# ZSHCRWY25/3DRVO-MARL-CollisionAvoidance

Measured on AMD Instinct MI355X. Metric: drone-steps/sec (env.step throughput), higher is better.
Workload: dtype f64; 1 GPU; BASELINE config 3 env.step: 64 drones x 4096 envs per GPU, nm=10, 0 buildings, map [50.0, 50.0, 10.0], fused step+auto-reset, f32 actions in HBM; envs_per_gpu=4096, drones=64, diag_build=False, cold_all=False, ablate=0, device_error_word=0

## Files before the change

### 3drvo-marl-collisionavoidance_amd/csrc/rvo3d_capi.hip

```cpp
#include "../../include/rvo3d.h"
#include "rvo3d_device.hpp"

#include <atomic>
#include <cmath>
#include <cstdio>
#include <cstdlib>
#include <cstring>
#include <exception>
#include <new>
#include <string>
#include <vector>

using rvo3d::Params;

namespace {
thread_local std::string g_err;

int fail(int code, const std::string& msg) {
  g_err = msg;
  return code;
}
#define HIP_TRY(expr)                                                            \
  do {                                                                           \
    hipError_t _e = (expr);                                                      \
    if (_e != hipSuccess)                                                        \
      return fail(RVO3D_ERR_HIP, std::string(#expr) + ": " + hipGetErrorString(_e)); \
  } while (0)

int api_caught(const char* what) noexcept {
  try {
    g_err = std::string("C++ exception: ") + what;
  } catch (...) {
    try { g_err.clear(); } catch (...) { }
  }
  return RVO3D_ERR_INVALID;
}
#define RVO3D_API_BEGIN try {
#define RVO3D_API_END                                              \
  }                                                                \
  catch (const std::exception& e) { return api_caught(e.what()); } \
  catch (...) { return api_caught("unknown"); }

inline size_t align_up(size_t x, size_t a) { return (x + a - 1) / a * a; }
volatile double kTwo = 2.0;
inline double py_sq(double x) { return std::pow(x, kTwo); }

double sq_threshold(double tau) {
  volatile double x = tau * tau;
  while (std::sqrt(std::nextafter((double)x, INFINITY)) <= tau) x = std::nextafter((double)x, INFINITY);
  while (std::sqrt((double)x) > tau) x = std::nextafter((double)x, -INFINITY);
  return x;
}
}

struct rvo3d_env {
  rvo3d_config cfg;
  Params P;
  rvo3d::Cold cold;
  void* arena = nullptr;
  size_t arena_bytes = 0;
  bool world_loaded = false;
  bool dv_valid = false;
  bool g_valid = false;
  int threads = 0, blocks = 0, lds = 0;
};

namespace {

int carve(rvo3d_env* h) {
  const rvo3d_config& c = h->cfg;
  const size_t EN = (size_t)c.num_envs * c.num_drones;
  const size_t S = align_up(EN, 64);
  Params& P = h->P;
  rvo3d::Cold& C = h->cold;
  P.S = (uint32_t)S;
  const size_t nf = Params::f64_arrays(c.max_points, c.neighbors_num);
  const size_t ni = Params::i32_arrays(c.neighbors_num, P.nw);
  struct Field { void** slot; size_t bytes; };
  std::vector<Field> f = {
      {(void**)&P.f64, nf * S * 8},
      {(void**)&P.i32, ni * S * 4},
      {(void**)&P.u8, 2 * S},
      {(void**)&C.bld, (size_t)(c.num_buildings > 0 ? c.num_buildings : 1) * 4 * 8},
      {(void**)&C.pow95, (size_t)c.max_points * 8},
      {(void**)&C.bgrid, (size_t)(C.bgx > 0 ? C.bgx * C.bgy : 1) * (rvo3d::kBgridK + 1) * 2},
      {(void**)&P.err, 256},
      {(void**)&P.cold_, sizeof(rvo3d::Cold)},
  };
  size_t total = 0;
  for (auto& x : f) total += align_up(x.bytes, 256);
  HIP_TRY(hipMalloc(&h->arena, total));
  HIP_TRY(hipMemset(h->arena, 0, total));
  h->arena_bytes = total;
  size_t off = 0;
  for (auto& x : f) {
    *x.slot = static_cast<char*>(h->arena) + off;
    off += align_up(x.bytes, 256);
  }
  HIP_TRY(hipMemcpy((void*)P.cold_, &C, sizeof C, hipMemcpyHostToDevice));
  return RVO3D_OK;
}

struct DeviceGuard {
  int prev = -1;
  bool changed = false;
  int enter(int dev) {
    hipError_t e = hipGetDevice(&prev);
    if (e == hipSuccess && prev != dev) {
      e = hipSetDevice(dev);
      changed = e == hipSuccess;
    }
    if (e != hipSuccess) return fail(RVO3D_ERR_HIP, std::string("hipSetDevice: ") + hipGetErrorString(e));
    return RVO3D_OK;
  }
  ~DeviceGuard() {
    if (changed) (void)hipSetDevice(prev);
  }
};

int check(rvo3d_env* h, bool need_world, DeviceGuard& g) {
  if (!h) return fail(RVO3D_ERR_INVALID, "null handle");
  if (need_world && !h->world_loaded)
    return fail(RVO3D_ERR_STATE, "rvo3d_load_world has not been called");
  return g.enter(h->cfg.device);
}

struct Pick { int nfix; bool pad; };
Pick pick_kernel(const Params& P) {
  if (P.nw == 1) {
    const int seg = (P.epb == 1 || P.epb == 2 || P.epb == 4) ? 64 / P.epb : 0;
    if (seg && P.N == seg) return {seg, false};
    if (seg >= 32 && P.N < seg) return {seg, true};
    return {0, false};
  }
  if (P.nw == 2) return {128, true};
  if (P.nw == 3) return {192, true};
  if (P.nw == 4) return {256, true};
  return {0, false};
}

template <int MODE, int NW, int NFIX, bool TRAIN, bool PAD>
void launch_inst(rvo3d_env* h, const Params& P, hipStream_t s) {
  hipLaunchKernelGGL((rvo3d::env_kernel<MODE, NW, NFIX, TRAIN, PAD>), dim3(h->blocks), dim3(h->threads), h->lds, s, P);
}
template <int MODE, int NW, int NFIX, bool PAD>
void launch_train(rvo3d_env* h, const Params& P, hipStream_t s) {
  if (P.env_train) launch_inst<MODE, NW, NFIX, true, PAD>(h, P, s);
  else launch_inst<MODE, NW, NFIX, false, PAD>(h, P, s);
}

template <int MODE, int NW>
int launch_nw(rvo3d_env* h, const Params& P, hipStream_t s) {
  const Pick k = pick_kernel(P);
  if constexpr (NW == 1) {
    if (k.nfix == 64) { if (k.pad) launch_train<MODE, 1, 64, true>(h, P, s); else launch_train<MODE, 1, 64, false>(h, P, s); }
    else if (k.nfix == 32) { if (k.pad) launch_train<MODE, 1, 32, true>(h, P, s); else launch_train<MODE, 1, 32, false>(h, P, s); }
    else if (k.nfix == 16) launch_train<MODE, 1, 16, false>(h, P, s);
    else launch_train<MODE, 1, 0, false>(h, P, s);
  } else if constexpr (NW == 2 || NW == 3 || NW == 4) {
    launch_train<MODE, NW, 64 * NW, true>(h, P, s);
  } else {
    launch_train<MODE, NW, 0, false>(h, P, s);
  }
  HIP_TRY(hipGetLastError());
  return RVO3D_OK;
}

template <int MODE>
int launch(rvo3d_env* h, const Params& P, hipStream_t s) {
  switch (P.nw) {
    case 1: return launch_nw<MODE, 1>(h, P, s);
    case 2: return launch_nw<MODE, 2>(h, P, s);
    case 3: return launch_nw<MODE, 3>(h, P, s);
    case 4: return launch_nw<MODE, 4>(h, P, s);
    default: return launch_nw<MODE, 8>(h, P, s);
  }
}

template <int MODE, int NW>
hipError_t allow_lds(int bytes) {
  hipError_t e = hipFuncSetAttribute((const void*)rvo3d::env_kernel<MODE, NW, 0, true, false>,
                                     hipFuncAttributeMaxDynamicSharedMemorySize, bytes);
  if (e != hipSuccess) return e;
  return hipFuncSetAttribute((const void*)rvo3d::env_kernel<MODE, NW, 0, false, false>,
                             hipFuncAttributeMaxDynamicSharedMemorySize, bytes);
}
template <int NW>
bool allow_lds_all(int bytes) {
  return allow_lds<rvo3d::kObserve, NW>(bytes) == hipSuccess &&
         allow_lds<rvo3d::kStep, NW>(bytes) == hipSuccess &&
         allow_lds<rvo3d::kStepAutoReset, NW>(bytes) == hipSuccess;
}

}

#ifndef RVO3D_MLP_WAVES
#define RVO3D_MLP_WAVES 8
#endif
namespace {
constexpr int kMlpWaves = RVO3D_MLP_WAVES;
template <auto Kernel>
int allow_dynamic_lds(int bytes) {
  static uint64_t attr_set = 0;
  int dev = 0;
  HIP_TRY(hipGetDevice(&dev));
  if (dev < 0 || dev >= 64 || !((attr_set >> dev) & 1)) {
    HIP_TRY(hipFuncSetAttribute(reinterpret_cast<const void*>(Kernel), hipFuncAttributeMaxDynamicSharedMemorySize, bytes));
    if (dev >= 0 && dev < 64) attr_set |= (uint64_t)1 << dev;
  }
  return RVO3D_OK;
}
template <bool X3, int KS1>
int launch_policy_mlp(const rvo3d::PolicyMlpArgs& A, unsigned grid, hipStream_t s) {
  constexpr auto kernel = X3 ? rvo3d::policy_mlp_x3_kernel<KS1, kMlpWaves> : rvo3d::policy_mlp_kernel<KS1, kMlpWaves>;
  constexpr int lds = X3 ? rvo3d::kX3LdsBytes : rvo3d::mlp_lds_bytes(KS1);
  if (int rc = allow_dynamic_lds<kernel>(lds)) return rc;
  hipLaunchKernelGGL(kernel, dim3(grid), dim3(64 * kMlpWaves), lds, s, A);
  HIP_TRY(hipGetLastError());
  return RVO3D_OK;
}
template <int H, int ND>
int launch_policy_rnn_tiles(const rvo3d::RnnTilesArgs& A, unsigned grid, hipStream_t s) {
  constexpr int lds = rvo3d::kRnnTilesWaves * H * 128;
  if (int rc = allow_dynamic_lds<rvo3d::policy_rnn_tiles_kernel<H, ND>>(lds)) return rc;
  hipLaunchKernelGGL((rvo3d::policy_rnn_tiles_kernel<H, ND>), dim3(grid), dim3(64 * rvo3d::kRnnTilesWaves), lds, s, A);
  HIP_TRY(hipGetLastError());
  return RVO3D_OK;
}
bool rnn_tiles_shape_ok(int32_t hidden, int32_t in_dim, int32_t state_dim) {
  return (hidden == 64 || hidden == 256) && in_dim == 9 && state_dim >= 1 && state_dim <= 16;
}

std::atomic<uint64_t*> g_step_dev{nullptr};

rvo3d::PolicySampleArgs sample_args(int32_t tanh_out, const float* log_std, float std_factor, uint64_t seed, uint64_t step,
                                    int64_t rows, float* act, float* logp, float* val, float* dbg_mu, float* dbg_raw) {
  rvo3d::PolicySampleArgs S{};
  S.tanh_out = tanh_out; S.log_std = log_std; S.std_factor = std_factor; S.seed = seed; S.step = step;
  S.step_dev = g_step_dev.load();
  S.rows = rows; S.act = act; S.logp = logp; S.val = val; S.dbg_mu = dbg_mu; S.dbg_raw = dbg_raw;
  return S;
}

template <class Args>
int copy_reader(Args& A, const rvo3d_rnn_policy& net) {
  if (!net.w_ih_f || !net.w_hh_f || !net.b_ih_f || !net.b_hh_f || !net.ln_w || !net.ln_b)
    return fail(RVO3D_ERR_INVALID, "null reader weight");
  const bool bi = net.w_ih_r != nullptr;
  if (bi != (net.w_hh_r != nullptr) || bi != (net.b_ih_r != nullptr) || bi != (net.b_hh_r != nullptr))
    return fail(RVO3D_ERR_INVALID, "the reverse direction needs all four of w_ih_r / w_hh_r / b_ih_r / b_hh_r");
  A.w_ih[0] = net.w_ih_f; A.w_hh[0] = net.w_hh_f; A.b_ih[0] = net.b_ih_f; A.b_hh[0] = net.b_hh_f;
  A.w_ih[1] = net.w_ih_r; A.w_hh[1] = net.w_hh_r; A.b_ih[1] = net.b_ih_r; A.b_hh[1] = net.b_hh_r;
  A.ln_w = net.ln_w; A.ln_b = net.ln_b; A.eps = net.ln_eps;
  return RVO3D_OK;
}
template <class Args>
int copy_heads(Args& A, const rvo3d_mlp_weights& pi, const rvo3d_mlp_weights& v, const char* missing) {
  const rvo3d_mlp_weights* n[2] = {&pi, &v};
  for (int i = 0; i < 2; ++i) {
    if (!n[i]->w1 || !n[i]->b1 || !n[i]->w2 || !n[i]->b2 || !n[i]->w3 || !n[i]->b3)
      return fail(RVO3D_ERR_INVALID, missing);
    A.w1[i] = n[i]->w1; A.b1[i] = n[i]->b1; A.w2[i] = n[i]->w2; A.b2[i] = n[i]->b2; A.w3[i] = n[i]->w3; A.b3[i] = n[i]->b3;
  }
  return RVO3D_OK;
}

template <bool X3>
int64_t mlp_net_bytes(int ks1) { return X3 ? rvo3d::mlp_x3_net_bytes(ks1) : rvo3d::mlp_net_bytes(ks1); }

template <bool X3>
int64_t policy_mlp_blob_bytes(int32_t obs_width) {
  if (obs_width < 1 || obs_width > 126) return -1;
  return 2 * mlp_net_bytes<X3>(rvo3d::mlp_ks1(obs_width));
}

template <bool X3>
int policy_mlp_pack(const rvo3d_mlp_weights* pi, const rvo3d_mlp_weights* v, int32_t obs_width, void* blob, void* stream) {
  if (!pi || !v || !blob) return fail(RVO3D_ERR_INVALID, "null pointer");
  if (obs_width < 1 || obs_width > 126) return fail(RVO3D_ERR_INVALID, "obs_width must be 1..126");
  if (reinterpret_cast<uintptr_t>(blob) & 15) return fail(RVO3D_ERR_INVALID, "blob must be 16-byte aligned");
  rvo3d::MlpPackArgs A;
  A.k_in = obs_width; A.ks1 = rvo3d::mlp_ks1(obs_width);
  if (int rc = copy_heads(A, *pi, *v, "null weight pointer")) return rc;
  A.blob = static_cast<unsigned char*>(blob);
  hipLaunchKernelGGL(X3 ? rvo3d::mlp_x3_pack_kernel : rvo3d::mlp_pack_kernel, dim3(64, 2), dim3(256), 0,
                     static_cast<hipStream_t>(stream), A);
  HIP_TRY(hipGetLastError());
  return RVO3D_OK;
}

template <bool X3>
int policy_mlp_sample(const void* blob, int32_t obs_width, const float* obs, int64_t obs_ld, int64_t rows,
                      const int32_t* vo_count, int32_t state_dim, int32_t row_dim, int32_t tanh_out, const float* log_std,
                      float std_factor, uint64_t seed, uint64_t step, float* act, float* logp, float* val, float* dbg_mu,
                      float* dbg_raw, void* stream) {
  if (!blob || !obs || !log_std || !act || !logp || !val) return fail(RVO3D_ERR_INVALID, "null pointer");
  if (obs_width < 1 || obs_width > 126) return fail(RVO3D_ERR_INVALID, "obs_width must be 1..126");
  if (rows < 0 || obs_ld < obs_width) return fail(RVO3D_ERR_INVALID, "rows < 0 or obs_ld < obs_width");
  if (rows > 0 && ((rows - 1) * obs_ld + obs_width) * 4 > (int64_t)0x7fffffff)
    return fail(RVO3D_ERR_INVALID, "the observation array must stay below 2 GiB per call (32-bit buffer offsets): split the rows");
  if (reinterpret_cast<uintptr_t>(obs) & 3) return fail(RVO3D_ERR_INVALID, "obs must be 4-byte aligned");
  if (reinterpret_cast<uintptr_t>(blob) & 15) return fail(RVO3D_ERR_INVALID, "blob must be 16-byte aligned");
  if (rows == 0) return RVO3D_OK;
  int dev = 0, cus = 0;
  HIP_TRY(hipGetDevice(&dev));
  HIP_TRY(hipDeviceGetAttribute(&cus, hipDeviceAttributeMultiprocessorCount, dev));
  const int ks1 = rvo3d::mlp_ks1(obs_width);
  rvo3d::PolicyMlpArgs A;
  A.blob = static_cast<const unsigned char*>(blob); A.net_bytes = mlp_net_bytes<X3>(ks1);
  A.obs = obs; A.ld_obs = obs_ld; A.k_in = obs_width;
  A.cnt = vo_count; A.state_dim = state_dim; A.row_dim = row_dim;
  if (vo_count && (state_dim < 0 || row_dim < 1 || state_dim > obs_width))
    return fail(RVO3D_ERR_INVALID, "vo_count needs 0 <= state_dim <= obs_width and row_dim >= 1");
  A.S = sample_args(tanh_out, log_std, std_factor, seed, step, rows, act, logp, val, dbg_mu, dbg_raw);
  const int64_t nchunks = (rows + 63) / 64;
  int64_t G = (nchunks + kMlpWaves - 1) / kMlpWaves;
  const int64_t Gmax = cus >= 2 ? cus / 2 : 1;
  if (G > Gmax) G = Gmax;
  const unsigned grid = (unsigned)(2 * G);
  hipStream_t s = static_cast<hipStream_t>(stream);
  switch (ks1) {
    case 1: return launch_policy_mlp<X3, 1>(A, grid, s);
    case 2: return launch_policy_mlp<X3, 2>(A, grid, s);
    case 3: return launch_policy_mlp<X3, 3>(A, grid, s);
    case 4: return launch_policy_mlp<X3, 4>(A, grid, s);
    case 5: return launch_policy_mlp<X3, 5>(A, grid, s);
    case 6: return launch_policy_mlp<X3, 6>(A, grid, s);
    case 7: return launch_policy_mlp<X3, 7>(A, grid, s);
    default: return launch_policy_mlp<X3, 8>(A, grid, s);
  }
}
}

extern "C" {

int rvo3d_version(void) { return RVO3D_VERSION; }
const char* rvo3d_last_error(void) { return g_err.c_str(); }

int rvo3d_create(const rvo3d_config* cfg, rvo3d_env** out) {
  RVO3D_API_BEGIN
  if (!cfg || !out) return fail(RVO3D_ERR_INVALID, "null argument");
  *out = nullptr;
  if (cfg->num_envs < 1 || cfg->num_drones < 1 || cfg->num_drones > rvo3d::kMaxThreads)
    return fail(RVO3D_ERR_INVALID, "need num_envs >= 1 and 1 <= num_drones <= 512");
  if (cfg->max_points < 2 || cfg->num_buildings < 0 || cfg->neighbors_num < 0)
    return fail(RVO3D_ERR_INVALID, "need max_points >= 2, num_buildings >= 0, neighbors_num >= 0");
  if ((long long)cfg->num_envs * cfg->num_drones > (1ll << 30))
    return fail(RVO3D_ERR_INVALID, "num_envs * num_drones too large");
  if (cfg->action_decimals > 9) return fail(RVO3D_ERR_INVALID, "action_decimals must be <= 9");
  DeviceGuard dg;
  if (int rc0 = dg.enter(cfg->device)) return rc0;

  rvo3d_env* h = new (std::nothrow) rvo3d_env();
  if (!h) return fail(RVO3D_ERR_INVALID, "out of host memory");
  struct Owner {
    rvo3d_env* p;
    ~Owner() {
      if (!p) return;
      if (p->arena) (void)hipFree(p->arena);
      delete p;
    }
  } owner{h};
  h->cfg = *cfg;
  Params& P = h->P;
  rvo3d::Cold& C = h->cold;
  std::memset(&P, 0, sizeof P);
  std::memset(&C, 0, sizeof C);
  P.E = cfg->num_envs; P.N = cfg->num_drones; P.P = cfg->max_points;
  C.nb = cfg->num_buildings; P.nm = cfg->neighbors_num; P.env_train = cfg->env_train ? 1 : 0;
  P.W = 12 + 9 * P.nm;
#ifdef RVO3D_DIAG
  if (const char* ab = std::getenv("RVO3D_ABLATE")) P.ablate = std::atoi(ab);
#endif
  C.act_scale = cfg->action_decimals >= 0 ? std::pow(10.0, cfg->action_decimals) : 0.0;
  for (int k = 0; k < 3; ++k) C.map[k] = cfg->map_size[k];
  P.T10 = sq_threshold(10.0);
  C.T5 = sq_threshold(5.0);
  C.bgx = C.bgy = 0; C.bg_inv = 0.0;
  if (cfg->num_buildings > 0 && cfg->map_size[0] > 0 && cfg->map_size[1] > 0 &&
      std::isfinite(cfg->map_size[0]) && std::isfinite(cfg->map_size[1])) {
    const double cs = std::fmax(8.0, std::fmax(cfg->map_size[0], cfg->map_size[1]) / 64.0);
    C.bgx = (int)std::ceil(cfg->map_size[0] / cs); C.bgy = (int)std::ceil(cfg->map_size[1] / cs);
    if (C.bgx < 1) C.bgx = 1;
    if (C.bgy < 1) C.bgy = 1;
    C.bg_inv = 1.0 / cs;
  }
  C.T04 = sq_threshold(0.4);
  {
    double mx = std::fmax(C.map[0], std::fmax(C.map[1], C.map[2]));
    if (!(mx > 0)) mx = 1.0;
    for (int k = 0; k < 3; ++k) C.cen[k] = 0.5 * C.map[k];
    const double cmax = 0.75 * mx + 16.0;
    const double u = std::ldexp(1.0, -24);
    const double eD = u * (2.0 * cmax + 21.0);
    const double band = 2.0 * (2.0 * 1.7320508 * 10.5 * eD + 3.0 * eD * eD + 8.0 * u * 110.25);
    C.cmax = (float)cmax;
    P.band = std::nextafter((float)band, INFINITY);
    const float t10f = std::nextafter((float)(P.T10 + band), INFINITY);
    P.t10n = -std::nextafter(t10f, INFINITY);
    P.bandn = P.band + P.t10n;
    C.kdot = std::nextafter((float)(2.0 * (eD + 4.0 * u * 10.5) * 1.001), INFINITY);
    const double gap = 512.0 * band;
    const double cs = 4.0 * (1.7320508 * eD / std::sqrt(gap) + 8.0 * u);
    P.x1_gap = (float)gap;
    P.x1_k2 = (float)(1.0 - (4e-3 + 4.0 * cs));
    const double cs_out = cs > 1e-3 ? cs : 1e-3;
    P.x1_cs2 = (float)(cs_out * cs_out);
  }

  const int N = P.N;
  int nw = (N + 63) / 64;
  P.nw = nw <= 4 ? nw : 8;
  int epb = P.nw == 1 ? 64 / N : 1;
  if (epb > P.E) epb = P.E;
  const int ring = (P.nw >= 2 && P.nw <= 4) ? 64 * P.nw : N;
  const int threads = P.nw == 1 ? 64 : (int)align_up((size_t)ring, 64);
  size_t lds = rvo3d::lds_bytes(threads, P.nm, epb, ring, P.nw);
#ifdef RVO3D_DIAG
  if (const char* pad = std::getenv("RVO3D_LDS_PAD")) lds += (size_t)std::atoi(pad);
#endif
  if (lds > 160 * 1024) {
    return fail(RVO3D_ERR_INVALID, "neighbors_num * num_drones needs more than 160 KiB of LDS");
  }
  P.epb = epb;
  C.zf_div = (uint32_t)((P.W & 1) == 0 ? (P.W - 12) / 2 : (P.W - 12));
  C.zf_magic = 0;
  if (C.zf_div > 0) {
    const uint32_t m = (uint32_t)(((1ull << 32) + C.zf_div - 1) / C.zf_div);
    bool ok = true;
    const uint64_t qmax = (uint64_t)threads * C.zf_div;
    for (uint64_t q = 0; q < qmax && ok; ++q) ok = ((q * m) >> 32) == q / C.zf_div;
    if (!ok) {
      return fail(RVO3D_ERR_INVALID, "neighbors_num too large for the zero-fill index trick");
    }
    C.zf_magic = m;
  }
  C.zf_q = (P.W & 1) == 0 ? (uint32_t)(P.W / 2) : 0u;
  C.zf_iters = 0;
  static_assert(rvo3d::kMaxThreads / 4 <= sizeof(C.zmask) / sizeof(C.zmask[0]),
                "Cold::zmask has one word per thread quad of the largest workgroup");
  std::memset(C.zmask, 0, sizeof C.zmask);
  {
    const uint32_t rb = 4u * (uint32_t)P.W;
    const uint32_t rows_full = (uint32_t)epb * (uint32_t)N, nwv = (uint32_t)threads / 64u;
    const uint32_t nblk = rows_full * rb >> 6;
    const uint32_t iters = (nblk + 16u * nwv - 1u) / (16u * nwv);
    if (C.zf_q != 0 && P.W >= 48 && (rows_full & 7u) == 0 && iters <= 32u) {
      for (uint32_t tq = 0; tq < (uint32_t)threads / 4u; ++tq) {
        uint32_t m = 0;
        for (uint32_t i = 0; i < iters; ++i) {
          const uint32_t blk = tq + 16u * nwv * i;
          if (blk >= nblk) break;
          const uint32_t o = (blk * 64u) % rb;
          if (o >= 48u && o + 64u <= rb) m |= 1u << i;
        }
        C.zmask[tq] = m;
      }
      C.zf_iters = (int)iters;
    }
  }
  h->threads = threads;
  h->blocks = (P.E + epb - 1) / epb;
  h->lds = (int)lds;
  if (lds > 64 * 1024) {
    const bool ok = P.nw == 1 ? allow_lds_all<1>((int)lds) : (P.nw == 8 && allow_lds_all<8>((int)lds));
    if (!ok) {
      return fail(RVO3D_ERR_HIP, "hipFuncSetAttribute(MaxDynamicSharedMemorySize) failed");
    }
  }
  int rc = carve(h);
  if (rc != RVO3D_OK) return rc;
  owner.p = nullptr;
  *out = h;
  return RVO3D_OK;
  RVO3D_API_END
}

int rvo3d_destroy(rvo3d_env* h) {
  RVO3D_API_BEGIN
  if (!h) return RVO3D_OK;
  DeviceGuard dg;
  (void)dg.enter(h->cfg.device);
  (void)hipDeviceSynchronize();
  if (h->arena) (void)hipFree(h->arena);
  delete h;
  return RVO3D_OK;
  RVO3D_API_END
}

int rvo3d_load_world(rvo3d_env* h, const double* waypoints, const int32_t* n_points,
                     const double* buildings, const double* radius, const double* priority,
                     void* stream) {
  RVO3D_API_BEGIN
  DeviceGuard dg;
  int rc = check(h, false, dg);
  if (rc) return rc;
  if (!waypoints || !n_points) return fail(RVO3D_ERR_INVALID, "waypoints / n_points are required");
  const Params& P = h->P;
  const rvo3d::Cold& C = h->cold;
  if (C.nb > 0 && !buildings) return fail(RVO3D_ERR_INVALID, "buildings required when num_buildings > 0");
  hipStream_t s = static_cast<hipStream_t>(stream);
  const size_t EN = (size_t)P.E * P.N;
  std::vector<double> wp((size_t)P.P * 3 * EN), rl(EN), rad(EN), pri(EN), p95(P.P);
  for (size_t g = 0; g < EN; ++g) {
    const int np = n_points[g];
    if (np < 2 || np > P.P) return fail(RVO3D_ERR_INVALID, "n_points entries must be in [2, max_points]");
    const double* src = waypoints + g * P.P * 3;
    double total = 0.0;
    for (int k = 0; k < P.P; ++k) {
      const int kk = k < np ? k : np - 1;
      for (int c = 0; c < 3; ++c) wp[((size_t)k * 3 + c) * EN + g] = src[kk * 3 + c];
      if (k + 1 < np) {
        const double dx = src[(k + 1) * 3] - src[k * 3], dy = src[(k + 1) * 3 + 1] - src[k * 3 + 1],
                     dz = src[(k + 1) * 3 + 2] - src[k * 3 + 2];
        total += std::sqrt(py_sq(dx) + py_sq(dy) + py_sq(dz));
      }
    }
    rl[g] = total;
    rad[g] = radius ? radius[g] : 0.2;
    pri[g] = priority ? priority[g] : 5.0;
  }
  {
    bool uni = true;
    for (size_t g = 1; g < EN && uni; ++g)
      uni = std::memcmp(&rad[g], &rad[0], 8) == 0 && std::memcmp(&pri[g], &pri[0], 8) == 0;
    h->P.uniform_rp = uni ? 1 : 0;
    h->P.r0 = rad[0];
    h->P.prio0 = pri[0];
  }
  for (int k = 0; k < P.P; ++k) p95[k] = std::pow(0.95, (double)k);
  HIP_TRY(hipMemcpy2DAsync((void*)P.wp(0, 0), (size_t)P.S * 8, wp.data(), EN * 8, EN * 8,
                           (size_t)P.P * 3, hipMemcpyHostToDevice, s));
  HIP_TRY(hipMemcpyAsync((void*)P.n_points(), n_points, EN * 4, hipMemcpyHostToDevice, s));
  HIP_TRY(hipMemcpyAsync((void*)P.route_len(), rl.data(), EN * 8, hipMemcpyHostToDevice, s));
  HIP_TRY(hipMemcpyAsync((void*)P.radius(), rad.data(), EN * 8, hipMemcpyHostToDevice, s));
  HIP_TRY(hipMemcpyAsync((void*)P.prio(), pri.data(), EN * 8, hipMemcpyHostToDevice, s));
  HIP_TRY(hipMemcpyAsync((void*)C.pow95, p95.data(), (size_t)P.P * 8, hipMemcpyHostToDevice, s));
  std::vector<uint16_t> grid;
  if (C.nb > 0) {
    HIP_TRY(hipMemcpyAsync((void*)C.bld, buildings, (size_t)C.nb * 32, hipMemcpyHostToDevice, s));
    if (C.bgx > 0) {
      const int K = rvo3d::kBgridK;
      const double cs = 1.0 / C.bg_inv;
      double rmax = 0.0;
      for (size_t g = 0; g < EN; ++g) {
        if (rad[g] != rad[g]) rmax = INFINITY;
        else if (rad[g] > rmax) rmax = rad[g];
      }
      grid.assign((size_t)C.bgx * C.bgy * (K + 1), 0);
      for (int ix = 0; ix < C.bgx; ++ix)
        for (int iy = 0; iy < C.bgy; ++iy) {
          uint16_t* cell = &grid[((size_t)ix * C.bgy + iy) * (K + 1)];
          const double x0 = ix == 0 ? -INFINITY : ix * cs, x1 = ix == C.bgx - 1 ? INFINITY : (ix + 1) * cs;
          const double y0 = iy == 0 ? -INFINITY : iy * cs, y1 = iy == C.bgy - 1 ? INFINITY : (iy + 1) * cs;
          int n = 0;
          bool overflow = false;
          for (int b = 0; b < C.nb && !overflow; ++b) {
            const double bx = buildings[4 * b], by = buildings[4 * b + 1];
            double reach = rmax + buildings[4 * b + 3];
            if (!(reach < 5.0)) reach = 5.0;
            reach += 1e-3;
            const double dx = bx < x0 ? x0 - bx : (bx > x1 ? bx - x1 : 0.0);
            const double dy = by < y0 ? y0 - by : (by > y1 ? by - y1 : 0.0);
            if (!(dx * dx + dy * dy > reach * reach)) {
              if (n == K || b > 0xfffe) overflow = true;
              else cell[1 + n++] = (uint16_t)b;
            }
          }
          cell[0] = overflow ? 0xffff : (uint16_t)n;
        }
      HIP_TRY(hipMemcpyAsync((void*)C.bgrid, grid.data(), grid.size() * 2, hipMemcpyHostToDevice, s));
    }
  }
  HIP_TRY(hipMemsetAsync(P.extra_len(), 0, EN * 8, s));
  const int tb = 256;
  hipLaunchKernelGGL(rvo3d::dv0_kernel, dim3((unsigned)((EN + tb - 1) / tb)), dim3(tb), 0, s, P);
  hipLaunchKernelGGL(rvo3d::reset_kernel, dim3((unsigned)((EN + tb - 1) / tb)), dim3(tb), 0, s, P,
                     (const uint8_t*)nullptr, (const uint8_t*)nullptr);
  hipLaunchKernelGGL(rvo3d::wpcache_kernel, dim3((unsigned)((EN + tb - 1) / tb)), dim3(tb), 0, s, P);
  HIP_TRY(hipGetLastError());
  HIP_TRY(hipStreamSynchronize(s));
  h->world_loaded = true;
  h->dv_valid = true;
  h->g_valid = false;
  return RVO3D_OK;
  RVO3D_API_END
}

int rvo3d_reset(rvo3d_env* h, const uint8_t* env_mask, void* stream) {
  RVO3D_API_BEGIN
  DeviceGuard dg;
  int rc = check(h, true, dg);
  if (rc) return rc;
  const size_t EN = (size_t)h->P.E * h->P.N;
  h->g_valid = false;
  hipLaunchKernelGGL(rvo3d::reset_kernel, dim3((unsigned)((EN + 255) / 256)), dim3(256), 0,
                     static_cast<hipStream_t>(stream), h->P, env_mask, (const uint8_t*)nullptr);
  HIP_TRY(hipGetLastError());
  return RVO3D_OK;
  RVO3D_API_END
}

int rvo3d_reset_drones(rvo3d_env* h, const uint8_t* drone_mask, void* stream) {
  RVO3D_API_BEGIN
  DeviceGuard dg;
  int rc = check(h, true, dg);
  if (rc) return rc;
  if (!drone_mask) return fail(RVO3D_ERR_INVALID, "drone_mask is required");
  const size_t EN = (size_t)h->P.E * h->P.N;
  h->g_valid = false;
  hipLaunchKernelGGL(rvo3d::reset_kernel, dim3((unsigned)((EN + 255) / 256)), dim3(256), 0,
                     static_cast<hipStream_t>(stream), h->P, (const uint8_t*)nullptr, drone_mask);
  HIP_TRY(hipGetLastError());
  return RVO3D_OK;
  RVO3D_API_END
}

int rvo3d_observe(rvo3d_env* h, float* obs, int32_t* vo_count, void* stream) {
  RVO3D_API_BEGIN
  DeviceGuard dg;
  int rc = check(h, true, dg);
  if (rc) return rc;
  if (!obs || !vo_count) return fail(RVO3D_ERR_INVALID, "obs / vo_count are required");
  Params P = h->P;
  P.obs = obs; P.vo_count = vo_count;
  P.zf16 = (h->cold.zf_q != 0 && (reinterpret_cast<uintptr_t>(obs) & 15) == 0 && P.nm > 0) ? 1 : 0;
  rc = launch<rvo3d::kObserve>(h, P, static_cast<hipStream_t>(stream));
  if (rc == RVO3D_OK) h->dv_valid = h->g_valid = true;
  return rc;
  RVO3D_API_END
}

static int step_common(rvo3d_env* h, const void* actions, int32_t action_dtype, float* obs,
                       int32_t* vo_count, float* reward, uint8_t* done, uint8_t* info,
                       uint8_t* finish, uint8_t* reset_mask, bool autoreset, void* stream,
                       const int32_t* prev_cnt = nullptr) {
  RVO3D_API_BEGIN
  DeviceGuard dg;
  int rc = check(h, true, dg);
  if (rc) return rc;
  if (!actions || !obs || !vo_count || !reward || !done || !info || !finish)
    return fail(RVO3D_ERR_INVALID, "null I/O pointer");
  if (action_dtype != RVO3D_F32 && action_dtype != RVO3D_F64)
    return fail(RVO3D_ERR_INVALID, "action_dtype must be RVO3D_F32 or RVO3D_F64");
  Params P = h->P;
  P.actions = actions; P.action_f64 = action_dtype == RVO3D_F64;
  P.obs = obs; P.vo_count = vo_count; P.reward = reward;
  P.zf16 = (h->cold.zf_q != 0 && (reinterpret_cast<uintptr_t>(obs) & 15) == 0 && P.nm > 0) ? 1 : 0;
  P.done = done; P.info = info; P.finish = finish; P.reset_mask = reset_mask;
  P.prev_cnt = prev_cnt;
  P.dv_cached = h->dv_valid ? 1 : 0;
  P.g_cached = h->g_valid ? 1 : 0;
  hipStream_t s = static_cast<hipStream_t>(stream);
  rc = autoreset ? launch<rvo3d::kStepAutoReset>(h, P, s) : launch<rvo3d::kStep>(h, P, s);
  if (rc == RVO3D_OK) h->dv_valid = h->g_valid = true;
  return rc;
  RVO3D_API_END
}

int rvo3d_step(rvo3d_env* h, const void* actions, int32_t action_dtype, float* obs,
               int32_t* vo_count, float* reward, uint8_t* done, uint8_t* info, uint8_t* finish,
               void* stream) {
  RVO3D_API_BEGIN
  return step_common(h, actions, action_dtype, obs, vo_count, reward, done, info, finish, nullptr,
                     false, stream);
  RVO3D_API_END
}

static int step_policy_common(rvo3d_env* h, const float* a_inc, float acceler, float* obs,
                              int32_t* vo_count, float* reward, uint8_t* done, uint8_t* info,
                              uint8_t* finish, uint8_t* reset_mask, bool autoreset, void* stream,
                              const int32_t* prev_cnt = nullptr) {
  RVO3D_API_BEGIN
  if (!h) return fail(RVO3D_ERR_INVALID, "null handle");
  h->P.action_mode = 1;
  h->P.acceler = acceler;
  const int rc = step_common(h, a_inc, RVO3D_F32, obs, vo_count, reward, done, info, finish,
                             reset_mask, autoreset, stream, prev_cnt);
  h->P.action_mode = 0;
  return rc;
  RVO3D_API_END
}

int rvo3d_step_policy(rvo3d_env* h, const float* a_inc, float acceler, float* obs,
                      int32_t* vo_count, float* reward, uint8_t* done, uint8_t* info,
                      uint8_t* finish, uint8_t* reset_mask, int32_t autoreset, void* stream) {
  RVO3D_API_BEGIN
  return step_policy_common(h, a_inc, acceler, obs, vo_count, reward, done, info, finish,
                            reset_mask, autoreset != 0, stream);
  RVO3D_API_END
}

int rvo3d_step_autoreset(rvo3d_env* h, const void* actions, int32_t action_dtype, float* obs,
                         int32_t* vo_count, float* reward, uint8_t* done, uint8_t* info,
                         uint8_t* finish, uint8_t* reset_mask, void* stream) {
  RVO3D_API_BEGIN
  return step_common(h, actions, action_dtype, obs, vo_count, reward, done, info, finish,
                     reset_mask, true, stream);
  RVO3D_API_END
}

int rvo3d_step_ex(rvo3d_env* h, const rvo3d_step_args* a, void* stream) {
  RVO3D_API_BEGIN
  if (!a) return fail(RVO3D_ERR_INVALID, "null argument");
  if (a->policy)
    return step_policy_common(h, static_cast<const float*>(a->actions), a->acceler, a->obs, a->vo_count, a->reward,
                              a->done, a->info, a->finish, a->reset_mask, a->autoreset != 0, stream,
                              a->prev_vo_count);
  return step_common(h, a->actions, a->action_dtype, a->obs, a->vo_count, a->reward, a->done, a->info, a->finish,
                     a->autoreset ? a->reset_mask : nullptr, a->autoreset != 0, stream, a->prev_vo_count);
  RVO3D_API_END
}

int rvo3d_policy_sample(const rvo3d_policy_heads* hd, int64_t rows, float std_factor, uint64_t seed,
                        uint64_t step, float* act, float* logp, float* val, float* dbg_mu, float* dbg_raw,
                        void* stream) {
  RVO3D_API_BEGIN
  if (!hd || !hd->h_pi || !hd->h_v || !hd->log_std || !act || !logp || !val)
    return fail(RVO3D_ERR_INVALID, "null pointer");
  if (rows < 0) return fail(RVO3D_ERR_INVALID, "rows < 0");
  if (rows == 0) return RVO3D_OK;
  rvo3d::PolicySampleArgs A = sample_args(hd->hidden == 0 ? 0 : hd->tanh_out,
                                          hd->log_std, std_factor, seed, step, rows, act, logp, val, dbg_mu, dbg_raw);
  A.h_pi = hd->h_pi; A.h_v = hd->h_v; A.ld_pi = hd->ld_pi; A.ld_v = hd->ld_v; A.hidden = hd->hidden;
  A.w_pi = hd->w_pi; A.b_pi = hd->b_pi; A.w_v = hd->w_v; A.b_v = hd->b_v;
  hipStream_t s = static_cast<hipStream_t>(stream);
  if (hd->hidden == 0) {
    if (hd->ld_pi < 3 || hd->ld_v < 1) return fail(RVO3D_ERR_INVALID, "hidden == 0 needs ld_pi >= 3 and ld_v >= 1");
    hipLaunchKernelGGL(rvo3d::policy_sample_direct_kernel, dim3((unsigned)((rows + 255) / 256)), dim3(256), 0, s, A);
  } else {
    if (!hd->w_pi || !hd->b_pi || !hd->w_v || !hd->b_v) return fail(RVO3D_ERR_INVALID, "head weights are required");
    const bool bf = hd->dtype == RVO3D_BF16;
    if (!bf && hd->dtype != RVO3D_F32) return fail(RVO3D_ERR_INVALID, "dtype must be RVO3D_F32 or RVO3D_BF16");
    const int per_chunk = bf ? 256 : 128;
    const int nch = hd->hidden / per_chunk;
    if (hd->hidden % per_chunk != 0 || (nch != 1 && nch != 2 && nch != 4 && nch != 8) || hd->hidden > 1024)
      return fail(RVO3D_ERR_INVALID, "hidden must be 128 / 256 / 512 / 1024 (float32) or 256 / 512 / 1024 (bfloat16)");
    const size_t es = bf ? 2 : 4;
    if (hd->ld_pi < hd->hidden || hd->ld_v < hd->hidden || (hd->ld_pi * es) % 16 || (hd->ld_v * es) % 16 ||
        (reinterpret_cast<uintptr_t>(hd->h_pi) & 15) || (reinterpret_cast<uintptr_t>(hd->h_v) & 15))
      return fail(RVO3D_ERR_INVALID, "hidden activations must be 16-byte aligned rows of at least `hidden` elements");
    const dim3 grid((unsigned)((rows + 127) / 128)), blk(256);
#define RVO3D_PS(T, N) hipLaunchKernelGGL((rvo3d::policy_sample_kernel<T, N>), grid, blk, 0, s, A)
    if (bf) {
      if (nch == 1) RVO3D_PS(rvo3d::bf16_t, 1); else if (nch == 2) RVO3D_PS(rvo3d::bf16_t, 2); else RVO3D_PS(rvo3d::bf16_t, 4);
    } else {
      if (nch == 1) RVO3D_PS(float, 1); else if (nch == 2) RVO3D_PS(float, 2); else if (nch == 4) RVO3D_PS(float, 4); else RVO3D_PS(float, 8);
    }
#undef RVO3D_PS
  }
  HIP_TRY(hipGetLastError());
  return RVO3D_OK;
  RVO3D_API_END
}

int64_t rvo3d_policy_mlp_blob_bytes(int32_t obs_width) { return policy_mlp_blob_bytes<false>(obs_width); }

int rvo3d_policy_mlp_pack(const rvo3d_mlp_weights* pi, const rvo3d_mlp_weights* v, int32_t obs_width, void* blob,
                          void* stream) {
  RVO3D_API_BEGIN
  return policy_mlp_pack<false>(pi, v, obs_width, blob, stream);
  RVO3D_API_END
}

int rvo3d_policy_mlp_sample(const void* blob, int32_t obs_width, const float* obs, int64_t obs_ld, int64_t rows,
                            const int32_t* vo_count, int32_t state_dim, int32_t row_dim, int32_t tanh_out, const float* log_std, float std_factor, uint64_t seed, uint64_t step,
                            float* act, float* logp, float* val, float* dbg_mu, float* dbg_raw, void* stream) {
  RVO3D_API_BEGIN
  return policy_mlp_sample<false>(blob, obs_width, obs, obs_ld, rows, vo_count, state_dim, row_dim, tanh_out, log_std,
                                  std_factor, seed, step, act, logp, val, dbg_mu, dbg_raw, stream);
  RVO3D_API_END
}

int64_t rvo3d_policy_mlp_x3_blob_bytes(int32_t obs_width) { return policy_mlp_blob_bytes<true>(obs_width); }

int rvo3d_policy_mlp_x3_pack(const rvo3d_mlp_weights* pi, const rvo3d_mlp_weights* v, int32_t obs_width, void* blob,
                             void* stream) {
  RVO3D_API_BEGIN
  return policy_mlp_pack<true>(pi, v, obs_width, blob, stream);
  RVO3D_API_END
}

int rvo3d_policy_mlp_x3_sample(const void* blob, int32_t obs_width, const float* obs, int64_t obs_ld, int64_t rows,
                               const int32_t* vo_count, int32_t state_dim, int32_t row_dim, int32_t tanh_out, const float* log_std, float std_factor, uint64_t seed, uint64_t step,
                               float* act, float* logp, float* val, float* dbg_mu, float* dbg_raw, void* stream) {
  RVO3D_API_BEGIN
  return policy_mlp_sample<true>(blob, obs_width, obs, obs_ld, rows, vo_count, state_dim, row_dim, tanh_out, log_std,
                                 std_factor, seed, step, act, logp, val, dbg_mu, dbg_raw, stream);
  RVO3D_API_END
}

int rvo3d_reader_zero_features(const float* obs, int64_t obs_ld, int64_t rows, int32_t state_dim, int32_t feat_dim,
                               const float* ln_w, const float* ln_b, float sum_h0, float sumsq_h0, float ln_eps,
                               float* out, int64_t out_ld, const int32_t* vo_count, int32_t* list, int32_t* count,
                               void* stream) {
  RVO3D_API_BEGIN
  if (!obs || !ln_w || !ln_b || !out) return fail(RVO3D_ERR_INVALID, "null pointer");
  if ((vo_count != nullptr) != (list != nullptr) || (vo_count != nullptr) != (count != nullptr))
    return fail(RVO3D_ERR_INVALID, "vo_count, list and count go together");
  if (state_dim < 1 || state_dim > rvo3d::kReaderMaxSd || feat_dim <= state_dim)
    return fail(RVO3D_ERR_INVALID, "need 1 <= state_dim <= 32 and feat_dim > state_dim");
  if (rows < 0 || obs_ld < (state_dim + 3) / 4 * 4 || out_ld < state_dim + 8)
    return fail(RVO3D_ERR_INVALID, "rows / row strides too small");
  if (rows == 0) return RVO3D_OK;
  rvo3d::ZeroFeatArgs A{obs, obs_ld, rows, state_dim, feat_dim, ln_w, ln_b, sum_h0, sumsq_h0, ln_eps, out, out_ld,
                        vo_count, list, count};
  hipLaunchKernelGGL(rvo3d::reader_zero_features_kernel, dim3((unsigned)((rows + 255) / 256)), dim3(256), 0,
                     static_cast<hipStream_t>(stream), A);
  HIP_TRY(hipGetLastError());
  return RVO3D_OK;
  RVO3D_API_END
}

int rvo3d_policy_rows(const rvo3d_rnn_policy* net, const float* obs, int64_t obs_ld, const int32_t* vo_count,
                      const int32_t* list, int32_t* count, int32_t* done_blocks, int32_t tanh_out, const float* log_std,
                      float std_factor, uint64_t seed, uint64_t step, float* act, float* logp, float* val, void* stream) {
  RVO3D_API_BEGIN
  if (!net || !obs || !vo_count || !list || !count || !done_blocks || !log_std || !act || !logp || !val)
    return fail(RVO3D_ERR_INVALID, "null pointer");
  rvo3d::PolicyRowsArgs A;
  if (int rc = copy_reader(A, *net)) return rc;
  if (net->hidden < 1 || net->hidden > 256 || net->in_dim < 1 || net->in_dim > rvo3d::kReaderMaxIn || net->state_dim < 1 ||
      net->state_dim > rvo3d::kReaderMaxSd || net->slots < 1 || net->slots > 16)
    return fail(RVO3D_ERR_INVALID, "hidden <= 256, in_dim <= 16, state_dim <= 32, slots <= 16");
  if (obs_ld < net->state_dim + net->slots * net->in_dim) return fail(RVO3D_ERR_INVALID, "obs_ld too small");
  if (int rc = copy_heads(A, net->pi, net->v, "null head weight")) return rc;
  A.obs = obs; A.obs_ld = obs_ld; A.cnt = vo_count; A.list = list; A.count = count; A.done_blocks = done_blocks;
  A.state_dim = net->state_dim; A.in_dim = net->in_dim; A.H = net->hidden; A.slots = net->slots;
  A.S = sample_args(tanh_out, log_std, std_factor, seed, step, 0, act, logp, val, nullptr, nullptr);
  hipLaunchKernelGGL(rvo3d::policy_rows_kernel, dim3(256), dim3(256), 0, static_cast<hipStream_t>(stream), A);
  HIP_TRY(hipGetLastError());
  return RVO3D_OK;
  RVO3D_API_END
}

int64_t rvo3d_policy_rnn_tiles_blob_bytes(int32_t hidden, int32_t in_dim, int32_t state_dim, int32_t bidir) {
  if (!rnn_tiles_shape_ok(hidden, in_dim, state_dim)) return -1;
  return rvo3d::rnn_tiles_layout(hidden, bidir ? 2 : 1).total;
}

int64_t rvo3d_policy_rnn_tiles_work_bytes(int64_t max_rows, int32_t slots) {
  if (max_rows < 1 || slots < 1 || slots > rvo3d::kRnnTilesMaxSlots) return -1;
  return 4 * (rvo3d::kRnnTilesWorkHeader + (int64_t)slots * max_rows);
}

int rvo3d_policy_rnn_tiles_pack(const rvo3d_rnn_policy* net, void* blob, int64_t blob_bytes, void* stream) {
  RVO3D_API_BEGIN
  if (!net || !blob) return fail(RVO3D_ERR_INVALID, "null pointer");
  rvo3d::RnnTilesPackArgs A;
  if (int rc = copy_reader(A, *net)) return rc;
  const bool bi = net->w_ih_r != nullptr;
  if (!rnn_tiles_shape_ok(net->hidden, net->in_dim, net->state_dim))
    return fail(RVO3D_ERR_INVALID, "rnn tiles: hidden must be 64 or 256, in_dim 9, state_dim 1..16");
  if (reinterpret_cast<uintptr_t>(blob) & 15) return fail(RVO3D_ERR_INVALID, "blob must be 16-byte aligned");
  if (blob_bytes != rvo3d_policy_rnn_tiles_blob_bytes(net->hidden, net->in_dim, net->state_dim, bi))
    return fail(RVO3D_ERR_INVALID, "blob_bytes does not match rvo3d_policy_rnn_tiles_blob_bytes for this shape");
  if (int rc = copy_heads(A, net->pi, net->v, "null head weight")) return rc;
  A.H = net->hidden; A.ND = bi ? 2 : 1; A.SD = net->state_dim; A.IN = net->in_dim;
  A.blob = static_cast<unsigned char*>(blob);
  hipLaunchKernelGGL(rvo3d::rnn_tiles_pack_kernel, dim3(128), dim3(256), 0, static_cast<hipStream_t>(stream), A);
  HIP_TRY(hipGetLastError());
  return RVO3D_OK;
  RVO3D_API_END
}

int rvo3d_policy_rnn_tiles(const void* blob, int64_t blob_bytes, int32_t hidden, int32_t in_dim, int32_t state_dim,
                           int32_t bidir, const float* obs, int64_t obs_ld, const int32_t* vo_count, const int32_t* list,
                           int32_t* count, int32_t* done_blocks, int32_t* work, int64_t max_rows, int32_t slots,
                           int32_t tanh_out, const float* log_std, float std_factor, uint64_t seed, uint64_t step,
                           float* act, float* logp, float* val, float* dbg_mu, void* stream) {
  RVO3D_API_BEGIN
  if (!blob || !obs || !vo_count || !list || !count || !done_blocks || !work || !log_std || !act || !logp || !val)
    return fail(RVO3D_ERR_INVALID, "null pointer");
  if (!rnn_tiles_shape_ok(hidden, in_dim, state_dim))
    return fail(RVO3D_ERR_INVALID, "rnn tiles: hidden must be 64 or 256, in_dim 9, state_dim 1..16");
  if (slots < 1 || slots > rvo3d::kRnnTilesMaxSlots) return fail(RVO3D_ERR_INVALID, "slots must be 1..12");
  if (blob_bytes != rvo3d_policy_rnn_tiles_blob_bytes(hidden, in_dim, state_dim, bidir))
    return fail(RVO3D_ERR_INVALID, "blob_bytes does not match this shape: the blob was packed for another one");
  if (reinterpret_cast<uintptr_t>(blob) & 15) return fail(RVO3D_ERR_INVALID, "blob must be 16-byte aligned");
  if (max_rows < 1 || max_rows > 0x7fffffff) return fail(RVO3D_ERR_INVALID, "max_rows must be 1..2^31-1");
  if (obs_ld < state_dim + slots * in_dim) return fail(RVO3D_ERR_INVALID, "obs_ld < state_dim + slots * in_dim");
  int dev = 0, cus = 0;
  HIP_TRY(hipGetDevice(&dev));
  HIP_TRY(hipDeviceGetAttribute(&cus, hipDeviceAttributeMultiprocessorCount, dev));
  rvo3d::RnnTilesArgs A;
  A.blob = static_cast<const unsigned char*>(blob);
  A.obs = obs; A.obs_ld = obs_ld; A.cnt = vo_count; A.list = list; A.count = count; A.done_blocks = done_blocks;
  A.work = work; A.max_rows = max_rows; A.SD = state_dim; A.slots = slots;
  A.S = sample_args(tanh_out, log_std, std_factor, seed, step, 0, act, logp, val, dbg_mu, nullptr);
  A.S.step_dev = nullptr;
  hipStream_t s = static_cast<hipStream_t>(stream);
  hipLaunchKernelGGL(rvo3d::rnn_tiles_bucket_kernel, dim3(256), dim3(256), 0, s, A);
  HIP_TRY(hipGetLastError());
  const unsigned grid = (unsigned)(cus > 0 ? cus : 1);
  if (hidden == 64) return bidir ? launch_policy_rnn_tiles<64, 2>(A, grid, s) : launch_policy_rnn_tiles<64, 1>(A, grid, s);
  return bidir ? launch_policy_rnn_tiles<256, 2>(A, grid, s) : launch_policy_rnn_tiles<256, 1>(A, grid, s);
  RVO3D_API_END
}

int rvo3d_reader_first_step(const rvo3d_gru_reader* rd, const float* obs, int64_t obs_ld, int64_t rows, void* feat,
                            int32_t feat_dtype, int64_t feat_ld, void* stream) {
  RVO3D_API_BEGIN
  if (!rd || !obs || !feat || !rd->w_ih_f || !rd->b_ih_f || !rd->b_hh_f || !rd->ln_w || !rd->ln_b)
    return fail(RVO3D_ERR_INVALID, "null pointer");
  if ((rd->w_ih_r != nullptr) != (rd->b_ih_r != nullptr) || (rd->w_ih_r != nullptr) != (rd->b_hh_r != nullptr))
    return fail(RVO3D_ERR_INVALID, "the reverse direction needs all three of w_ih_r / b_ih_r / b_hh_r");
  if (rd->hidden < 64 || rd->hidden > 256 || rd->hidden % 64 != 0 || rd->in_dim != 9 || rd->state_dim < 0 ||
      rd->state_dim > rvo3d::kReaderMaxSd)
    return fail(RVO3D_ERR_INVALID, "hidden must be 64 / 128 / 192 / 256, in_dim 9, state_dim <= 32");
  if (feat_dtype != RVO3D_F32 && feat_dtype != RVO3D_BF16) return fail(RVO3D_ERR_INVALID, "feat_dtype must be RVO3D_F32 or RVO3D_BF16");
  if (rows < 0 || obs_ld < rd->state_dim + rd->in_dim || feat_ld < rd->state_dim + rd->hidden)
    return fail(RVO3D_ERR_INVALID, "rows / row strides too small");
  if (feat_dtype == RVO3D_BF16 && ((reinterpret_cast<uintptr_t>(feat) & 7) || (feat_ld & 3)))
    return fail(RVO3D_ERR_INVALID, "bf16 features: feat 8-byte aligned, feat_ld a multiple of 4");
  if (rows == 0) return RVO3D_OK;
  rvo3d::ReaderArgs A;
  A.w_ih_f = rd->w_ih_f; A.b_ih_f = rd->b_ih_f; A.b_hh_f = rd->b_hh_f;
  A.w_ih_r = rd->w_ih_r; A.b_ih_r = rd->b_ih_r; A.b_hh_r = rd->b_hh_r;
  A.ln_w = rd->ln_w; A.ln_b = rd->ln_b; A.H = rd->hidden; A.IN = rd->in_dim; A.SD = rd->state_dim; A.eps = rd->ln_eps;
  A.obs = obs; A.obs_ld = obs_ld; A.rows = rows; A.feat = feat; A.feat_bf16 = feat_dtype == RVO3D_BF16; A.feat_ld = feat_ld;
  const int64_t groups = (rows + rvo3d::kReaderRows - 1) / rvo3d::kReaderRows;
  const unsigned grid = (unsigned)(groups < 256 * 8 ? groups : 256 * 8);
  hipLaunchKernelGGL((rvo3d::reader_first_step_kernel<9>), dim3(grid), dim3((unsigned)rd->hidden), 0,
                     static_cast<hipStream_t>(stream), A);
  HIP_TRY(hipGetLastError());
  return RVO3D_OK;
  RVO3D_API_END
}

int rvo3d_rollout_set_step_counter(uint64_t* device_counter) {
  RVO3D_API_BEGIN
  g_step_dev.store(device_counter);
  return RVO3D_OK;
  RVO3D_API_END
}

int rvo3d_rollout_account(int32_t E, int32_t N, const float* reward, const uint8_t* done, const uint8_t* finish,
                          int32_t sanitize, int32_t max_ep_len, int32_t epoch_end, float* rew_slot, float* ep_ret,
                          int32_t* ep_len, uint8_t* cut_slot, uint8_t* extra_mask, double* sums, int32_t* any_extra,
                          void* stream) {
  RVO3D_API_BEGIN
  if (E < 1 || N < 1 || N > rvo3d::kMaxThreads) return fail(RVO3D_ERR_INVALID, "need num_envs >= 1 and 1 <= num_drones <= 512");
  if (!reward || !done || !finish || !rew_slot || !ep_ret || !ep_len || !cut_slot || !extra_mask || !sums || !any_extra)
    return fail(RVO3D_ERR_INVALID, "null pointer");
  rvo3d::AccountArgs A{E, N, reward, done, finish, sanitize, max_ep_len, epoch_end, rew_slot, ep_ret, ep_len,
                       cut_slot, extra_mask, sums, any_extra, g_step_dev.load()};
  hipLaunchKernelGGL(rvo3d::rollout_account_kernel, dim3((unsigned)E), dim3((unsigned)align_up((size_t)N, 64)), 0,
                     static_cast<hipStream_t>(stream), A);
  HIP_TRY(hipGetLastError());
  return RVO3D_OK;
  RVO3D_API_END
}

int rvo3d_gae(const float* rew, const float* val, const uint8_t* cut, int64_t steps, int64_t envs, int64_t drones,
              double gamma, double lam, float* adv, float* ret, void* stream) {
  RVO3D_API_BEGIN
  if (!rew || !val || !cut || !adv || !ret) return fail(RVO3D_ERR_INVALID, "null pointer");
  if (steps < 1 || envs < 1 || drones < 1) return fail(RVO3D_ERR_INVALID, "need steps >= 1, envs >= 1 and drones >= 1");
  if (!std::isfinite(gamma) || !std::isfinite(lam)) return fail(RVO3D_ERR_INVALID, "gamma and lam must be finite");
  const int64_t kMaxColumns = (int64_t)0x7fffffff * 256, kMaxElems = (int64_t)1 << 58;
  if (envs > kMaxColumns / drones || steps > kMaxElems / (envs * drones))
    return fail(RVO3D_ERR_INVALID, "steps * envs * drones too large");
  const uint64_t n4 = (uint64_t)steps * (uint64_t)envs * (uint64_t)drones * 4, n1 = (uint64_t)steps * (uint64_t)envs;
  auto overlap = [](const void* a, uint64_t an, const void* b, uint64_t bn) {
    const uintptr_t x = reinterpret_cast<uintptr_t>(a), y = reinterpret_cast<uintptr_t>(b);
    return x < y + bn && y < x + an;
  };
  if (overlap(adv, n4, rew, n4) || overlap(adv, n4, val, n4) || overlap(adv, n4, cut, n1) ||
      overlap(ret, n4, rew, n4) || overlap(ret, n4, val, n4) || overlap(ret, n4, cut, n1) || overlap(adv, n4, ret, n4))
    return fail(RVO3D_ERR_INVALID, "adv / ret overlap an input or each other: the outputs need storage of their own");
  const int64_t columns = envs * drones;
  rvo3d::GaeArgs A{rew, val, cut, steps, envs, drones, gamma, gamma * lam, adv, ret};
  hipLaunchKernelGGL(rvo3d::gae_kernel, dim3((unsigned)((columns + 255) / 256)), dim3(256), 0,
                     static_cast<hipStream_t>(stream), A);
  HIP_TRY(hipGetLastError());
  return RVO3D_OK;
  RVO3D_API_END
}

int rvo3d_set_reward_f64(rvo3d_env* h, double* reward64) {
  RVO3D_API_BEGIN
  if (!h) return fail(RVO3D_ERR_INVALID, "null handle");
  h->P.reward64 = reward64;
  return RVO3D_OK;
  RVO3D_API_END
}

int rvo3d_des_vel(rvo3d_env* h, double* des_vel, void* stream) {
  RVO3D_API_BEGIN
  DeviceGuard dg;
  int rc = check(h, true, dg);
  if (rc) return rc;
  if (!des_vel) return fail(RVO3D_ERR_INVALID, "des_vel is required");
  const size_t EN = (size_t)h->P.E * h->P.N;
  hipLaunchKernelGGL(rvo3d::des_vel_kernel, dim3((unsigned)((EN + 255) / 256)), dim3(256), 0,
                     static_cast<hipStream_t>(stream), h->P, des_vel);
  HIP_TRY(hipGetLastError());
  return RVO3D_OK;
  RVO3D_API_END
}

int rvo3d_rvo_vel(rvo3d_env* h, const double* vmax, double acceler, double* out_vel, void* stream) {
  RVO3D_API_BEGIN
  DeviceGuard dg;
  int rc = check(h, true, dg);
  if (rc) return rc;
  if (!vmax || !out_vel) return fail(RVO3D_ERR_INVALID, "vmax / out_vel are required");
  if (!(acceler >= 0.0 && acceler <= 1.0))
    return fail(RVO3D_ERR_INVALID, "acceler must be in [0, 1] (at most 4 candidates per axis)");
  rvo3d::RvoVelArgs A;
  for (int k = 0; k < 3; ++k) A.vmax[k] = vmax[k];
  A.acceler = acceler;
  const int T = (int)align_up((size_t)h->P.N, 64);
  hipLaunchKernelGGL(rvo3d::rvo_vel_kernel, dim3((unsigned)h->P.E), dim3((unsigned)T),
                     (size_t)T * 8 * sizeof(double), static_cast<hipStream_t>(stream), h->P, A, out_vel);
  HIP_TRY(hipGetLastError());
  return RVO3D_OK;
  RVO3D_API_END
}

int rvo3d_state_ptrs(rvo3d_env* h, rvo3d_state_view* out) {
  RVO3D_API_BEGIN
  if (!h || !out) return fail(RVO3D_ERR_INVALID, "null argument");
  const Params& P = h->P;
  out->px = P.px(); out->py = P.py(); out->pz = P.pz(); out->vx = P.vx(); out->vy = P.vy(); out->vz = P.vz();
  out->yaw = P.yaw(); out->pitch = P.pitch(); out->real_len = P.real_len(); out->max_dev = P.max_dev();
  out->extra_len = P.extra_len(); out->wp_idx = P.wp_idx(); out->arrive = P.arrive(); out->dest = P.dest();
  return RVO3D_OK;
  RVO3D_API_END
}

int rvo3d_get_state(rvo3d_env* h, double* pos, double* vel, double* yaw, double* pitch,
                    double* real_len, double* max_dev, double* extra_len, int32_t* wp_idx,
                    uint8_t* arrive, uint8_t* dest, void* stream) {
  RVO3D_API_BEGIN
  DeviceGuard dg;
  int rc = check(h, true, dg);
  if (rc) return rc;
  const Params& P = h->P;
  hipStream_t s = static_cast<hipStream_t>(stream);
  const int EN = P.E * P.N;
  const dim3 grid((EN + 255) / 256), blk(256);
  if (pos) hipLaunchKernelGGL(rvo3d::soa_to_aos3, grid, blk, 0, s, P.px(), P.py(), P.pz(), pos, EN);
  if (vel) hipLaunchKernelGGL(rvo3d::soa_to_aos3, grid, blk, 0, s, P.vx(), P.vy(), P.vz(), vel, EN);
  HIP_TRY(hipGetLastError());
  const hipMemcpyKind k = hipMemcpyDeviceToDevice;
  if (yaw) HIP_TRY(hipMemcpyAsync(yaw, P.yaw(), (size_t)EN * 8, k, s));
  if (pitch) HIP_TRY(hipMemcpyAsync(pitch, P.pitch(), (size_t)EN * 8, k, s));
  if (real_len) HIP_TRY(hipMemcpyAsync(real_len, P.real_len(), (size_t)EN * 8, k, s));
  if (max_dev) HIP_TRY(hipMemcpyAsync(max_dev, P.max_dev(), (size_t)EN * 8, k, s));
  if (extra_len) HIP_TRY(hipMemcpyAsync(extra_len, P.extra_len(), (size_t)EN * 8, k, s));
  if (wp_idx) HIP_TRY(hipMemcpyAsync(wp_idx, P.wp_idx(), (size_t)EN * 4, k, s));
  if (arrive) HIP_TRY(hipMemcpyAsync(arrive, P.arrive(), (size_t)EN, k, s));
  if (dest) HIP_TRY(hipMemcpyAsync(dest, P.dest(), (size_t)EN, k, s));
  return RVO3D_OK;
  RVO3D_API_END
}

int rvo3d_set_state(rvo3d_env* h, const double* pos, const double* vel, const double* yaw,
                    const double* pitch, const double* real_len, const double* max_dev,
                    const double* extra_len, const int32_t* wp_idx, const uint8_t* arrive,
                    const uint8_t* dest, void* stream) {
  RVO3D_API_BEGIN
  DeviceGuard dg;
  int rc = check(h, true, dg);
  if (rc) return rc;
  h->dv_valid = h->g_valid = false;
  const Params& P = h->P;
  hipStream_t s = static_cast<hipStream_t>(stream);
  const int EN = P.E * P.N;
  const dim3 grid((EN + 255) / 256), blk(256);
  if (pos) hipLaunchKernelGGL(rvo3d::aos3_to_soa, grid, blk, 0, s, pos, P.px(), P.py(), P.pz(), EN);
  if (vel) hipLaunchKernelGGL(rvo3d::aos3_to_soa, grid, blk, 0, s, vel, P.vx(), P.vy(), P.vz(), EN);
  HIP_TRY(hipGetLastError());
  const hipMemcpyKind k = hipMemcpyDeviceToDevice;
  if (yaw) HIP_TRY(hipMemcpyAsync(P.yaw(), yaw, (size_t)EN * 8, k, s));
  if (pitch) HIP_TRY(hipMemcpyAsync(P.pitch(), pitch, (size_t)EN * 8, k, s));
  if (real_len) HIP_TRY(hipMemcpyAsync(P.real_len(), real_len, (size_t)EN * 8, k, s));
  if (max_dev) HIP_TRY(hipMemcpyAsync(P.max_dev(), max_dev, (size_t)EN * 8, k, s));
  if (extra_len) HIP_TRY(hipMemcpyAsync(P.extra_len(), extra_len, (size_t)EN * 8, k, s));
  if (wp_idx) {
    HIP_TRY(hipMemcpyAsync(P.wp_idx(), wp_idx, (size_t)EN * 4, k, s));
    hipLaunchKernelGGL(rvo3d::wpcache_kernel, grid, blk, 0, s, P);
  }
  if (arrive) HIP_TRY(hipMemcpyAsync(P.arrive(), arrive, (size_t)EN, k, s));
  if (dest) HIP_TRY(hipMemcpyAsync(P.dest(), dest, (size_t)EN, k, s));
  return RVO3D_OK;
  RVO3D_API_END
}

int rvo3d_error_flags(rvo3d_env* h, uint32_t* flags, void* stream) {
  RVO3D_API_BEGIN
  DeviceGuard dg;
  int rc = check(h, false, dg);
  if (rc) return rc;
  if (!flags) return fail(RVO3D_ERR_INVALID, "flags is required");
  hipStream_t s = static_cast<hipStream_t>(stream);
  HIP_TRY(hipMemcpyAsync(flags, h->P.err, 4, hipMemcpyDeviceToHost, s));
  HIP_TRY(hipMemsetAsync(h->P.err, 0, 4, s));
  HIP_TRY(hipStreamSynchronize(s));
  return RVO3D_OK;
  RVO3D_API_END
}

#ifdef RVO3D_DIAG
int rvo3d_debug_stamps(rvo3d_env* h, unsigned long long* stamps) {
  RVO3D_API_BEGIN
  if (!h) return fail(RVO3D_ERR_INVALID, "null handle");
  h->P.dbg = stamps;
  return RVO3D_OK;
  RVO3D_API_END
}
#endif

int rvo3d_kernel_name(rvo3d_env* h, int32_t mode, char* buf, int32_t cap) {
  RVO3D_API_BEGIN
  if (!h || !buf || cap < 1) return fail(RVO3D_ERR_INVALID, "null handle / buffer");
  if (mode < 0 || mode > 2) return fail(RVO3D_ERR_INVALID, "mode: 0 observe, 1 step, 2 step + auto-reset");
  const Pick k = pick_kernel(h->P);
  std::snprintf(buf, (size_t)cap, "rvo3d::env_kernel<%d, %d, %d, %s, %s>", (int)mode, h->P.nw, k.nfix,
                h->P.env_train ? "true" : "false", k.pad ? "true" : "false");
  return RVO3D_OK;
  RVO3D_API_END
}

int rvo3d_launch_info(rvo3d_env* h, int32_t* threads, int32_t* envs_per_block, int32_t* blocks,
                      int32_t* lds_bytes) {
  RVO3D_API_BEGIN
  if (!h) return fail(RVO3D_ERR_INVALID, "null handle");
  if (threads) *threads = h->threads;
  if (envs_per_block) *envs_per_block = h->P.epb;
  if (blocks) *blocks = h->blocks;
  if (lds_bytes) *lds_bytes = h->lds;
  return RVO3D_OK;
  RVO3D_API_END
}

}
```

### 3drvo-marl-collisionavoidance_amd/csrc/rvo3d_math.hpp

```cpp
#pragma once

#include "rvo3d_params.hpp"

namespace rvo3d {

__device__ __forceinline__ double sq(double x) { return x * x; }
__device__ __forceinline__ double dot3b(double ax, double ay, double az, double bx,
                                        double by, double bz) {
  return __builtin_fma(az, bz, __builtin_fma(ay, by, ax * bx));
}
__device__ __forceinline__ double norm3b(double x, double y, double z) {
  return __builtin_sqrt(dot3b(x, y, z, x, y, z));
}
__device__ __forceinline__ double norm2sq(double x, double y) { return __builtin_fma(y, y, x * x); }
__device__ __forceinline__ bool finite_d(double q) { return __builtin_fabs(q) < __builtin_inf(); }

__device__ __forceinline__ float round2_f32(double x) {
  const double k = __builtin_rint(x * 100.0);
  return __builtin_fabs(k) < 16777216.0 ? (float)(k * 0.01) : (float)(k / 100.0);
}
__device__ __forceinline__ double k_over_1000(double k) {
  const double q = k * 0.001;
  const double r = __builtin_fma(-q, 1000.0, k);
  const double c = q + r * 0.001;
  return finite_d(k) ? c : k;
}

constexpr uint32_t kDvInvalid = 0xffffffffu;
__device__ __forceinline__ void dv_encode(const double dv[3], uint32_t& a, uint32_t& b) {
  const double k0 = __builtin_rint(dv[0] * 1000.0), k1 = __builtin_rint(dv[1] * 1000.0),
               k2 = __builtin_rint(dv[2] * 1000.0);
  const bool ok = __builtin_fabs(k0) <= 1023.0 && __builtin_fabs(k1) <= 1023.0 &&
                  __builtin_fabs(k2) <= 1023.0 && k_over_1000(k0) == dv[0] &&
                  k_over_1000(k1) == dv[1] && k_over_1000(k2) == dv[2];
  const uint32_t nz = (uint32_t)(k0 == 0.0 && __builtin_signbit(dv[0])) |
                      ((uint32_t)(k1 == 0.0 && __builtin_signbit(dv[1])) << 1) |
                      ((uint32_t)(k2 == 0.0 && __builtin_signbit(dv[2])) << 2);
  a = ok ? ((uint32_t)((int)k0 + 1024) | ((uint32_t)((int)k1 + 1024) << 16)) : kDvInvalid;
  b = (uint32_t)((int)(ok ? k2 : 0.0) + 1024) | (nz << 16);
}
__device__ __forceinline__ bool dv_decode(uint32_t a, uint32_t b, double dv[3]) {
  if (a == kDvInvalid) return false;
  const int k0 = (int)(a & 0xffffu) - 1024, k1 = (int)(a >> 16) - 1024, k2 = (int)(b & 0xffffu) - 1024;
  dv[0] = (b & (1u << 16)) ? -0.0 : k_over_1000((double)k0);
  dv[1] = (b & (1u << 17)) ? -0.0 : k_over_1000((double)k1);
  dv[2] = (b & (1u << 18)) ? -0.0 : k_over_1000((double)k2);
  return true;
}

__device__ __forceinline__ double py_round2_c(double x) {
  double p = x * 100.0;
  double e = __builtin_fma(x, 100.0, -p);
  double c = __builtin_floor(p);
  double d = (p - (c + 0.5)) + e;
  if (d > 0.0) c += 1.0;
  else if (d == 0.0 && (((long long)c) & 1)) c += 1.0;
  return c;
}
__device__ __forceinline__ double clampd(double x, double lo, double hi) {
  return x < lo ? lo : (x > hi ? hi : x);
}
__device__ __forceinline__ double np_mod(double a, double b) {
  double m;
  if (b > 0.0 && a > -b && a < 2.0 * b) m = a >= b ? a - b : a;
  else m = fmod(a, b);
  if (m != 0.0) {
    if ((b < 0.0) != (m < 0.0)) m += b;
  } else {
    m = __builtin_copysign(0.0, b);
  }
  return m;
}

__device__ __forceinline__ void des_vel(const Params& P, const double p[3], const double cur[3],
                                        double out[3]) {
  const double dx = cur[0] - p[0], dy = cur[1] - p[1], dz = cur[2] - p[2];
  const double d2 = dot3b(dx, dy, dz, dx, dy, dz);
  if (d2 > P.cold().T04) {
    const double inv = 1000.0 / __builtin_sqrt(d2);
    const double ux = dx * inv, uy = dy * inv, uz = dz * inv;
    double kx = __builtin_rint(ux), ky = __builtin_rint(uy), kz = __builtin_rint(uz);
    const double m = __builtin_fmin(__builtin_fmin(0.5 - __builtin_fabs(ux - kx),
                                                   0.5 - __builtin_fabs(uy - ky)),
                                    0.5 - __builtin_fabs(uz - kz));
    if (!(m > 1e-7)) {
      const double az = atan2(dy, dx);
      const double el = atan2(dz, __builtin_sqrt(norm2sq(dx, dy)));
      double sa, ca, se, ce;
      sincos(az, &sa, &ca);
      sincos(el, &se, &ce);
      kx = __builtin_rint((1.0 * (ca * ce)) * 1000.0);
      ky = __builtin_rint((1.0 * (sa * ce)) * 1000.0);
      kz = __builtin_rint((1.0 * se) * 1000.0);
    }
    out[0] = k_over_1000(kx); out[1] = k_over_1000(ky); out[2] = k_over_1000(kz);
  } else {
    out[0] = out[1] = out[2] = 0.0;
  }
}

__device__ __forceinline__ double deviation(const double a[3], const double b[3],
                                            const double p[3]) {
  double dx = b[0] - a[0], dy = b[1] - a[1], dz = b[2] - a[2];
  double mag = __builtin_sqrt(sq(dx) + sq(dy) + sq(dz));
  if (mag == 0.0) return 0.0;
  double hx = dx / mag, hy = dy / mag, hz = dz / mag;
  double qx0 = p[0] - a[0], qy0 = p[1] - a[1], qz0 = p[2] - a[2];
  double t = qx0 * hx + qy0 * hy + qz0 * hz;
  double qx = a[0] + t * hx, qy = a[1] + t * hy, qz = a[2] + t * hz;
  return __builtin_sqrt(sq(p[0] - qx) + sq(p[1] - qy) + sq(p[2] - qz));
}

__device__ __forceinline__ bool arrived(const Params& P, const double p[3], const double d[3]) {
  const double x = p[0] - d[0], y = p[1] - d[1], z = p[2] - d[2];
  return dot3b(x, y, z, x, y, z) <= P.cold().T04;
}

__device__ __forceinline__ double vo_exp_time(double rx, double ry, double rz, double rvx,
                                              double rvy, double rvz, double ra, double rb) {
  double r = ra + rb;
  double ux = -rvx, uy = -rvy, uz = -rvz;
  double a = sq(ux) + sq(uy) + sq(uz);
  double b = 2 * rx * ux + 2 * ry * uy + 2 * rz * uz;
  double c = sq(rx) + sq(ry) + sq(rz) - sq(r);
  if (c <= 0) return 0.0;
  double temp = sq(b) - 4 * a * c;
  if (temp <= 0) return __builtin_inf();
  double s = __builtin_sqrt(temp);
  double t1 = (-b + s) / (2 * a);
  double t2 = (-b - s) / (2 * a);
  if (t1 < 0 && t2 < 0) return -1.0;
  double t3 = t1 >= 0 ? t1 : __builtin_inf();
  double t4 = t2 >= 0 ? t2 : __builtin_inf();
  return t4 < t3 ? t4 : t3;
}

struct Drone {
  double x, y, z, vx, vy, vz, r, prio;
};

struct PairOut {
  bool collision, flag;
  double t, iet, md;
  int alpha_c;
};

}
```

### 3drvo-marl-collisionavoidance_amd/csrc/rvo3d_pairs.hpp

```cpp
#pragma once

#include <type_traits>

#include "rvo3d_lds.hpp"

namespace rvo3d {

__device__ __forceinline__ double pair_md(const Drone& S, const Drone& O) {
  double rx = O.x - S.x, ry = O.y - S.y, rz = O.z - S.z;
  return __builtin_sqrt(sq(ry) + sq(rx) + sq(rz)) - O.r;
}

template <bool TRAIN>
__device__ __forceinline__ PairOut pair_eval(const Params& P, const Drone& S, const Lds& L, int k,
                                             const double a[3]) {
  PairOut o;
  o.flag = false; o.collision = false; o.t = 0.0; o.iet = 0.0; o.md = 0.0; o.alpha_c = 0;
  const double rx = L.x[k] - S.x, ry = L.y[k] - S.y, rz = L.z[k] - S.z;
  const double d2 = dot3b(rx, ry, rz, rx, ry, rz);
  if (!(d2 <= P.T10)) return o;
  if (d2 == 0.0 && rx == 0.0 && ry == 0.0 && rz == 0.0) return o;
  const double Or = L.r[k];
  const double ssum = sq(ry) + sq(rx) + sq(rz);
  const double R = S.r + Or;
  const double thr = TRAIN ? R : (S.r - kExpRadius + Or);
  const double thr2 = thr * thr;
  bool coll;
  if (ssum < thr2 * (1.0 - 1e-15)) coll = thr >= 0;
  else if (ssum > thr2 * (1.0 + 1e-15)) coll = false;
  else coll = __builtin_sqrt(ssum) <= thr;
  if (coll) { o.collision = true; return o; }
  const double dotp = S.vx * rx + S.vy * ry + S.vz * rz;
  if (dotp <= 0) return o;
  if (!TRAIN && d2 < R * R * (1.0 + 1e-12)) {
    const double R2 = R * R;
    if (d2 < R2 * (1.0 - 1e-15) || (d2 < R2 * (1.0 + 1e-15) && __builtin_sqrt(d2) < R)) {
      atomicOr(P.err, 2u);
      return o;
    }
  }
  const double Ovx = L.vx[k], Ovy = L.vy[k], Ovz = L.vz[k], Oprio = L.prio[k];
  const double pr = (S.prio == Oprio) ? 0.5 : S.prio / (S.prio + Oprio);
  const double paax = pr * (2 * S.x + (S.vx + Ovx));
  const double paay = pr * (2 * S.y + (S.vy + Ovy));
  const double paaz = pr * (2 * S.z + (S.vz + Ovz));
  const double wx = (S.x + 2 * a[0]) - paax, wy = (S.y + 2 * a[1]) - paay,
               wz = (S.z + 2 * a[2]) - paaz;
  const double dp = dot3b(rx, ry, rz, wx, wy, wz);
  if (dp <= 0) return o;
  const double w2 = dot3b(wx, wy, wz, wx, wy, wz);
  const double K = kCosD * (double)__builtin_sqrtf((float)(d2 - R * R)) - kSinD * R;
  if (K > 0 && dp * dp < (w2 * (K * K)) * (1.0 - 1e-5)) return o;
  const double nab = __builtin_sqrt(d2);
  const double alpha_c = py_round2_c(asin(R / nab));
  const double AB = nab * __builtin_sqrt(w2);
  const double cosang = (AB != 0) ? dp / AB : 0.0;
  const double beta_c = __builtin_rint(acos(cosang) * 100.0);
  if (!(alpha_c > beta_c)) return o;
  const double rvx = 2 * a[0] - Ovx - S.vx, rvy = 2 * a[1] - Ovy - S.vy,
               rvz = 2 * a[2] - Ovz - S.vz;
  const double t = vo_exp_time(rx, ry, rz, rvx, rvy, rvz, S.r, Or);
  if (t < kCtimeThreshold) {
    o.flag = true;
    o.t = t;
    o.iet = 1 / (t + 0.2);
    o.md = __builtin_sqrt(ssum) - Or;
    o.alpha_c = (int)alpha_c;
  }
  return o;
}

__device__ __forceinline__ int insert_row(const Params& P, const Lds& L, int g, int lbase,
                                          const Drone& S, const PairOut& po, int j, int kept) {
  const size_t T = P.S;
  asm volatile("" : "+v"(g));
  double* const iet = P.row_iet(0) + g;
  uint32_t* const pk = P.row_pk(0) + g;
  int pos = kept;
  for (int s = 0; s < kept; ++s) {
    const double ie = iet[s * T];
    bool new_first;
    if (po.iet != ie) new_first = po.iet < ie;
    else {
      const int js = (int)(pk[s * T] & 0xffffu);
      const double mds = pair_md(S, lds_drone(L, lbase + js));
      new_first = (po.md != mds) ? (po.md > mds) : (j < js);
    }
    if (new_first) { pos = s; break; }
  }
  const uint32_t packed = ((uint32_t)po.alpha_c << 16) | (uint32_t)j;
  if (kept < P.nm) {
    for (int s = kept; s > pos; --s) {
      iet[s * T] = iet[(s - 1) * T];
      pk[s * T] = pk[(s - 1) * T];
    }
    iet[pos * T] = po.iet;
    pk[pos * T] = packed;
    ++kept;
  } else if (pos > 0) {
    for (int s = 0; s < pos - 1; ++s) {
      iet[s * T] = iet[(s + 1) * T];
      pk[s * T] = pk[(s + 1) * T];
    }
    iet[(pos - 1) * T] = po.iet;
    pk[(pos - 1) * T] = packed;
  }
  return kept;
}

template <int NW>
__device__ __forceinline__ int mi(const Lds& L, int slot, int w) {
  return NW == 1 ? slot : w * L.T + slot;
}

enum { WX = 0, WY, WZ, WVX, WVY, WVZ, WR, WKD, WAX, WAY, WAZ, WPRIO };

template <int NW>
__device__ __forceinline__ void stage_f32(const Params& P, const Lds& L, int el, int d,
                                          bool active, const double p[3], const double v[3],
                                          const double az[3], double r, double prio) {
  if (!active) return;
  const double cx = p[0] - P.cold().cen[0], cy = p[1] - P.cold().cen[1], cz = p[2] - P.cold().cen[2];
  const float fvx = (float)v[0], fvy = (float)v[1], fvz = (float)v[2];
  const bool vzero = v[0] == 0.0 && v[1] == 0.0 && v[2] == 0.0;
  const float val[12] = {(float)cx, (float)cy, (float)cz, fvx, fvy, fvz, (float)r,
                         vzero ? -1.0f
                               : P.cold().kdot * (__builtin_fabsf(fvx) + __builtin_fabsf(fvy) + __builtin_fabsf(fvz)) + 1e-30f,
                         (float)az[0], (float)az[1], (float)az[2], (float)prio};
  const int o = el * 2 * P.N + d, os = el * P.N + d;
#pragma unroll
  for (int k = 0; k < 12; ++k) {
    if (k == WX || k == WY || k == WZ || k == WR) {
      L.w[k][o] = val[k];
      if (NW == 1 || d <= (P.N >> 1)) L.w[k][o + P.N] = val[k];
    } else L.w[k][os] = val[k];
  }
  const double cm = (double)P.cold().cmax;
  if (!(__builtin_fabs(cx) <= cm && __builtin_fabs(cy) <= cm && __builtin_fabs(cz) <= cm))
    L.far[el] = 1;
}

template <int NW>
__device__ __forceinline__ void valid_offsets(int N, int d, uint32_t valid[NW]) {
  const int H = N >> 1;
#pragma unroll
  for (int w = 0; w < NW; ++w) {
    const int n = H - 32 * w;
    valid[w] = n >= 32 ? 0xffffffffu : (n > 0 ? ((1u << n) - 1u) : 0u);
  }
  if (!(N & 1) && d >= H && H > 0) {
#pragma unroll
    for (int w = 0; w < NW; ++w)
      if (((H - 1) >> 5) == w) valid[w] &= ~(1u << ((H - 1) & 31));
  }
}

__device__ __forceinline__ float gate_acc(float dx, float dy, float dz, float t10n) {
  return __builtin_fmaf(dz, dz, __builtin_fmaf(dy, dy, __builtin_fmaf(dx, dx, t10n)));
}
__device__ __forceinline__ uint32_t shift_in_sign(uint32_t m, float acc) {
  return __builtin_amdgcn_alignbit(m, __builtin_bit_cast(uint32_t, acc), 31);
}

#ifndef RVO3D_G_UNROLL
#define RVO3D_G_UNROLL 8
#endif
template <bool TOUCHONLY, bool UNIFORM_R = false>
__device__ __forceinline__ uint32_t gate_word(const Params& P, const Lds& L, int o0, int w, int H,
                                              float mex, float mey, float mez, float mer,
                                              uint32_t* range_out = nullptr) {
  typedef float v2f __attribute__((ext_vector_type(2)));
  const v2f sx = {mex, mex}, sy = {mey, mey}, sz = {mez, mez}, sr = {mer, mer};
  const v2f tn = {P.t10n, P.t10n};
  const int kend = (H - 32 * w) < 32 ? (H - 32 * w) : 32;
  uint32_t mr = 0u, mt = 0u;
  const v2f ru = sr + sr;
  const v2f rcu = __builtin_elementwise_fma(ru * ru, (v2f){1.00001f, 1.00001f},
                                            (v2f){P.bandn, P.bandn});
#pragma unroll RVO3D_G_UNROLL
  for (int b = (kend - 1) & ~1; b >= 0; b -= 2) {
    const int o = o0 + 32 * w + b + 1;
    const v2f dx = (v2f){L.w[WX][o], L.w[WX][o + 1]} - sx;
    const v2f dy = (v2f){L.w[WY][o], L.w[WY][o + 1]} - sy;
    const v2f dz = (v2f){L.w[WZ][o], L.w[WZ][o + 1]} - sz;
    v2f acc = __builtin_elementwise_fma(dx, dx, tn);
    acc = __builtin_elementwise_fma(dy, dy, acc);
    acc = __builtin_elementwise_fma(dz, dz, acc);
    mr = shift_in_sign(shift_in_sign(mr, acc.y), acc.x);
    if (TOUCHONLY) {
      v2f rc = rcu;
      if (!UNIFORM_R) {
        const v2f rs = (v2f){L.w[WR][o], L.w[WR][o + 1]} + sr;
        rc = __builtin_elementwise_fma(rs * rs, (v2f){1.00001f, 1.00001f},
                                       (v2f){P.bandn, P.bandn});
      }
      const v2f at = acc - rc;
      mt = shift_in_sign(shift_in_sign(mt, at.y), at.x);
    }
  }
  if (TOUCHONLY) {
    if (range_out) *range_out = mr;
    return mt & mr;
  }
  return mr;
}

#ifndef RVO3D_GS_UNROLL
#define RVO3D_GS_UNROLL 4
#endif
template <int NW, bool TOUCH, bool UNIFORM_R>
__device__ __forceinline__ void gate_words_shared(const Params& P, const Lds& L, int d) {
  typedef float v2f __attribute__((ext_vector_type(2)));
  constexpr int N = 64 * NW;
  const v2f tn = {P.t10n, P.t10n};
  v2f ox[NW], oy[NW], oz[NW], orr[NW], rcu[NW];
  uint32_t mr[NW], mt[NW];
  int own[NW];
#pragma unroll
  for (int s = 0; s < NW; ++s) {
    int e = d - 32 * s;
    if (e < 0) e += N;
    own[s] = e;
    const float x = L.w[WX][e], y = L.w[WY][e], z = L.w[WZ][e], r = L.w[WR][e];
    ox[s] = (v2f){x, x}; oy[s] = (v2f){y, y}; oz[s] = (v2f){z, z}; orr[s] = (v2f){r, r};
    const v2f ru = orr[s] + orr[s];
    rcu[s] = __builtin_elementwise_fma(ru * ru, (v2f){1.00001f, 1.00001f}, (v2f){P.bandn, P.bandn});
    mr[s] = 0u; mt[s] = 0u;
  }
#pragma unroll RVO3D_GS_UNROLL
  for (int b = 30; b >= 0; b -= 2) {
    const int o = d + b + 1;
    const v2f X = {L.w[WX][o], L.w[WX][o + 1]}, Y = {L.w[WY][o], L.w[WY][o + 1]},
              Z = {L.w[WZ][o], L.w[WZ][o + 1]};
    v2f R = {0.f, 0.f};
    if (TOUCH && !UNIFORM_R) R = (v2f){L.w[WR][o], L.w[WR][o + 1]};
#pragma unroll
    for (int s = 0; s < NW; ++s) {
      const v2f dx = X - ox[s], dy = Y - oy[s], dz = Z - oz[s];
      v2f acc = __builtin_elementwise_fma(dx, dx, tn);
      acc = __builtin_elementwise_fma(dy, dy, acc);
      acc = __builtin_elementwise_fma(dz, dz, acc);
      mr[s] = shift_in_sign(shift_in_sign(mr[s], acc.y), acc.x);
      if (TOUCH) {
        v2f rc = rcu[s];
        if (!UNIFORM_R) {
          const v2f rs = R + orr[s];
          rc = __builtin_elementwise_fma(rs * rs, (v2f){1.00001f, 1.00001f}, (v2f){P.bandn, P.bandn});
        }
        const v2f at = acc - rc;
        mt[s] = shift_in_sign(shift_in_sign(mt[s], at.y), at.x);
      }
    }
  }
#pragma unroll
  for (int s = 0; s < NW; ++s)
    L.mask2[mi<NW>(L, own[s], s)] =
        (unsigned long long)mr[s] | ((unsigned long long)(TOUCH ? (mt[s] & mr[s]) : 0u) << 32);
}

template <int CW> struct OffsetSet;
template <> struct OffsetSet<1> {
  uint32_t a;
  __device__ __forceinline__ static OffsetSet load(const uint32_t* g) { return {g[0]}; }
  __device__ __forceinline__ static OffsetSet none() { return {0u}; }
  __device__ __forceinline__ bool any() const { return a != 0u; }
  __device__ __forceinline__ int lowest() const { return __builtin_ctz(a); }
  __device__ __forceinline__ void drop() { a &= a - 1u; }
  __device__ __forceinline__ void add(int b, int on) { a |= (uint32_t)(on & 1) << b; }
  __device__ __forceinline__ void store(uint32_t* g) const { g[0] = a; }
  __device__ __forceinline__ int count() const { return __builtin_popcount(a); }
};
template <> struct OffsetSet<2> {
  unsigned long long a;
  __device__ __forceinline__ static OffsetSet load(const uint32_t* g) {
    return {(unsigned long long)g[0] | ((unsigned long long)g[1] << 32)};
  }
  __device__ __forceinline__ static OffsetSet none() { return {0ull}; }
  __device__ __forceinline__ bool any() const { return a != 0ull; }
  __device__ __forceinline__ int lowest() const { return __builtin_ctzll(a); }
  __device__ __forceinline__ void drop() { a &= a - 1ull; }
  __device__ __forceinline__ void add(int b, int on) { a |= (unsigned long long)(on & 1) << b; }
  __device__ __forceinline__ void store(uint32_t* g) const { g[0] = (uint32_t)a; g[1] = (uint32_t)(a >> 32); }
  __device__ __forceinline__ int count() const { return __builtin_popcountll(a); }
};
template <> struct OffsetSet<3> {
  unsigned long long lo;
  uint32_t hi;
  __device__ __forceinline__ static OffsetSet load(const uint32_t* g) {
    return {(unsigned long long)g[0] | ((unsigned long long)g[1] << 32), g[2]};
  }
  __device__ __forceinline__ static OffsetSet none() { return {0ull, 0u}; }
  __device__ __forceinline__ bool any() const { return lo != 0ull || hi != 0u; }
  __device__ __forceinline__ int lowest() const { return lo != 0ull ? __builtin_ctzll(lo) : 64 + __builtin_ctz(hi); }
  __device__ __forceinline__ void drop() {
    if (lo != 0ull) lo &= lo - 1ull; else hi &= hi - 1u;
  }
  __device__ __forceinline__ void add(int b, int on) {
    if (b < 64) lo |= (unsigned long long)(on & 1) << b; else hi |= (uint32_t)(on & 1) << (b - 64);
  }
  __device__ __forceinline__ void store(uint32_t* g) const { g[0] = (uint32_t)lo; g[1] = (uint32_t)(lo >> 32); g[2] = hi; }
  __device__ __forceinline__ int count() const { return __builtin_popcountll(lo) + __builtin_popcount(hi); }
};
template <> struct OffsetSet<4> {
  unsigned long long lo, hi;
  __device__ __forceinline__ static OffsetSet load(const uint32_t* g) {
    return {(unsigned long long)g[0] | ((unsigned long long)g[1] << 32),
            (unsigned long long)g[2] | ((unsigned long long)g[3] << 32)};
  }
  __device__ __forceinline__ static OffsetSet none() { return {0ull, 0ull}; }
  __device__ __forceinline__ bool any() const { return (lo | hi) != 0ull; }
  __device__ __forceinline__ int lowest() const {
    return lo != 0ull ? __builtin_ctzll(lo) : 64 + __builtin_ctzll(hi);
  }
  __device__ __forceinline__ void drop() {
    if (lo != 0ull) lo &= lo - 1ull; else hi &= hi - 1ull;
  }
  __device__ __forceinline__ void add(int b, int on) {
    const unsigned long long v = (unsigned long long)(on & 1) << (b & 63);
    if (b < 64) lo |= v; else hi |= v;
  }
  __device__ __forceinline__ void store(uint32_t* g) const {
    g[0] = (uint32_t)lo; g[1] = (uint32_t)(lo >> 32); g[2] = (uint32_t)hi; g[3] = (uint32_t)(hi >> 32);
  }
  __device__ __forceinline__ int count() const { return __builtin_popcountll(lo) + __builtin_popcountll(hi); }
};

typedef float v2f __attribute__((ext_vector_type(2)));

struct X1End { v2f x, y, z, r, vx, vy, vz, kd, prio; };
struct X1Bits { bool pi0, pj0, pi1, pj1, keep0, keep1; };

template <bool TOUCH, bool ZERO>
__device__ __forceinline__ X1Bits x1_pairs(const Params& P, bool far, const X1End& me, const X1End& o, v2f tax,
                                           v2f tay, v2f taz, v2f aox, v2f aoy, v2f aoz) {
  const v2f dx = o.x - me.x, dy = o.y - me.y, dz = o.z - me.z;
  const v2f d2 = __builtin_elementwise_fma(dz, dz, __builtin_elementwise_fma(dy, dy, dx * dx));
  const v2f rs = o.r + me.r;
  const v2f rs2 = rs * rs;
  const v2f tch = __builtin_elementwise_fma(rs2, (v2f){1.00001f, 1.00001f}, (v2f){P.band, P.band});
  const v2f vi = __builtin_elementwise_fma(me.vz, dz, __builtin_elementwise_fma(me.vy, dy, me.vx * dx));
  const v2f vj = __builtin_elementwise_fma(o.vz, dz, __builtin_elementwise_fma(o.vy, dy, o.vx * dx));
  const v2f gap = d2 - rs2;
  const v2f sq_ = {__builtin_amdgcn_sqrtf(__builtin_fmaxf(gap.x, 0.f)),
                   __builtin_amdgcn_sqrtf(__builtin_fmaxf(gap.y, 0.f))};
  const v2f Kr = (v2f){0.999998f, 0.999998f} * sq_ - (v2f){2.0e-3f, 2.0e-3f} * rs;
  const v2f K = {__builtin_fmaxf(Kr.x, 0.f), __builtin_fmaxf(Kr.y, 0.f)};
  const v2f K2 = K * K * (v2f){P.x1_k2, P.x1_k2};
  const v2f hx = me.vx + o.vx, hy = me.vy + o.vy, hz = me.vz + o.vz;
  const v2f wix = tax - hx, wiy = tay - hy, wiz = taz - hz;
  const v2f dpi = __builtin_elementwise_fma(dz, wiz, __builtin_elementwise_fma(dy, wiy, dx * wix));
  const v2f wi2 = __builtin_elementwise_fma(wiz, wiz, __builtin_elementwise_fma(wiy, wiy, wix * wix));
  v2f dpj, wj2;
  if (ZERO) {
    dpj = -dpi;
    wj2 = wi2;
  } else {
    const v2f four2 = {4.f, 4.f};
    const v2f wjx = four2 * aox - hx, wjy = four2 * aoy - hy, wjz = four2 * aoz - hz;
    dpj = -__builtin_elementwise_fma(dz, wjz, __builtin_elementwise_fma(dy, wjy, dx * wjx));
    wj2 = __builtin_elementwise_fma(wjz, wjz, __builtin_elementwise_fma(wjy, wjy, wjx * wjx));
  }
  const v2f cs = (v2f){P.x1_cs2, P.x1_cs2} * d2;
  const v2f si = dpi * __builtin_elementwise_abs(dpi), sj = dpj * __builtin_elementwise_abs(dpj);
  const v2f ci = -(cs * wi2), cj = -(cs * wj2), ki = wi2 * K2, kj = wj2 * K2;
  X1Bits b;
#define RVO3D_X1_HALF(c, pi, pj, kp)                                                          \
  {                                                                                           \
                 \
    const bool touch = TOUCH & (d2.c <= tch.c);                                               \
    const bool ai = vi.c > -me.kd.c, aj = vj.c < o.kd.c;                                      \
    const bool filt = (gap.c >= P.x1_gap) & (o.prio.c == me.prio.c);                          \
    const bool oi = si.c < (si.c < 0.f ? ci.c : ki.c);                                        \
    const bool oj = sj.c < (sj.c < 0.f ? cj.c : kj.c);                                        \
    pi = far | touch | (ai & !(filt & oi));                                                   \
    pj = far | touch | (aj & !(filt & oj));                                                   \
    kp = far | ai | aj;                                                                       \
  }
  RVO3D_X1_HALF(x, b.pi0, b.pj0, b.keep0)
  RVO3D_X1_HALF(y, b.pi1, b.pj1, b.keep1)
#undef RVO3D_X1_HALF
  return b;
}

__device__ __forceinline__ int wave_prefix_sum(int v) {
  v += __builtin_amdgcn_update_dpp(0, v, 0x111, 0xf, 0xf, false);
  v += __builtin_amdgcn_update_dpp(0, v, 0x112, 0xf, 0xf, false);
  v += __builtin_amdgcn_update_dpp(0, v, 0x114, 0xf, 0xf, false);
  v += __builtin_amdgcn_update_dpp(0, v, 0x118, 0xf, 0xf, false);
  v += __builtin_amdgcn_update_dpp(0, v, 0x142, 0xa, 0xf, false);
  v += __builtin_amdgcn_update_dpp(0, v, 0x143, 0xc, 0xf, false);
  return v;
}

struct X1Idx {
  int s0, s1, kb0, kb1, d0, d1, oa0, oa1, ob0, ob1, jd0, jd1, j0, j1;
  __device__ __forceinline__ X1Idx(uint32_t e, int N) {
    s0 = (int)(e & 63u); s1 = (int)((e >> 16) & 63u);
    kb0 = (int)((e >> 6) & 31u); kb1 = (int)((e >> 22) & 31u);
    d0 = s0 & (N - 1); d1 = s1 & (N - 1);
    oa0 = 2 * s0 - d0; oa1 = 2 * s1 - d1;
    ob0 = oa0 + kb0 + 1; ob1 = oa1 + kb1 + 1;
    jd0 = (d0 + kb0 + 1) & (N - 1); jd1 = (d1 + kb1 + 1) & (N - 1);
    j0 = s0 - d0 + jd0; j1 = s1 - d1 + jd1;
  }
};

template <bool ROWS, bool TOUCH>
__device__ __forceinline__ bool x1_queue(const Params& P, const Lds& L, int lane, int N, bool active, bool far,
                                         bool act0, uint32_t cand) {
  typedef uint32_t __attribute__((may_alias)) u32a;
  if (!active) cand = 0u;
  const int c = __builtin_popcount(cand);
  const int incl = wave_prefix_sum(c);
  const int total = __builtin_amdgcn_readlane(incl, 63);
  if (total > kX1Queue || __ballot(active && far) != 0ull) return false;
  for (int pos = incl - c; cand; cand &= cand - 1u, ++pos)
    L.x1q[pos] = (uint16_t)((uint32_t)lane | ((uint32_t)__builtin_ctz(cand) << 6));
  __syncthreads();
  const bool zero = ROWS && __ballot(active && !act0) == 0ull;
  for (int base = 0; base < total; base += 128) {
    const int i0 = base + 2 * lane;
    const bool on0 = i0 < total, on1 = i0 + 1 < total;
    uint32_t e = *reinterpret_cast<const u32a*>(L.x1q + i0);
    X1Bits b;
    {
      const X1Idx k(e, N);
#define RVO3D_LD2(K, F) ((v2f){L.w[K][k.F##0], L.w[K][k.F##1]})
      const X1End me = {RVO3D_LD2(WX, oa), RVO3D_LD2(WY, oa), RVO3D_LD2(WZ, oa), RVO3D_LD2(WR, oa), RVO3D_LD2(WVX, s),
                        RVO3D_LD2(WVY, s), RVO3D_LD2(WVZ, s), RVO3D_LD2(WKD, s), RVO3D_LD2(WPRIO, s)};
      const X1End o = {RVO3D_LD2(WX, ob), RVO3D_LD2(WY, ob), RVO3D_LD2(WZ, ob), RVO3D_LD2(WR, ob), RVO3D_LD2(WVX, j),
                       RVO3D_LD2(WVY, j), RVO3D_LD2(WVZ, j), RVO3D_LD2(WKD, j), RVO3D_LD2(WPRIO, j)};
      const v2f z2 = {0.f, 0.f};
      if (zero) {
        b = x1_pairs<TOUCH, true>(P, false, me, o, z2, z2, z2, z2, z2, z2);
      } else {
        const v2f four2 = {4.f, 4.f};
        b = x1_pairs<TOUCH, false>(P, false, me, o, four2 * RVO3D_LD2(WAX, s), four2 * RVO3D_LD2(WAY, s),
                                   four2 * RVO3D_LD2(WAZ, s), RVO3D_LD2(WAX, j), RVO3D_LD2(WAY, j), RVO3D_LD2(WAZ, j));
      }
#undef RVO3D_LD2
    }
    if (N != 64) asm volatile("" : "+v"(e));
    const X1Idx k(e, N);
    if (b.pi0 & on0) atomicOr(&L.mask2[k.s0], 1ull << k.jd0);
    if (b.pi1 & on1) atomicOr(&L.mask2[k.s1], 1ull << k.jd1);
    if (b.pj0 & on0) atomicOr(&L.mask2[k.j0], 1ull << k.d0);
    if (b.pj1 & on1) atomicOr(&L.mask2[k.j1], 1ull << k.d1);
    if (ROWS) {
      if (b.keep0 & on0) atomicOr(&L.x1keep[k.s0], 1u << k.kb0);
      if (b.keep1 & on1) atomicOr(&L.x1keep[k.s1], 1u << k.kb1);
    }
  }
  return true;
}

template <int NW, bool ROWS, bool TOUCH, bool TRAIN, bool GSHARE = false, bool QUEUE = false>
__device__ __forceinline__ int sweep_env(const Params& P, const Lds& L, int lane, int el, int d,
                                         int g, bool active, const Drone& S, const double a[3],
                                         bool zero_act, bool act0, bool& flag, double& tmin,
                                         bool& collision, uint32_t gw[NW], bool have_gw) {
  flag = false;
  tmin = __builtin_inf();
  int kept = 0;
  const int N = P.N, H = N >> 1;
  if (GSHARE && !have_gw) {
    const bool far = L.far[el] != 0;
    if (!far) gate_words_shared<NW, false, false>(P, L, d);
    __syncthreads();
    if (active) {
      uint32_t valid[NW];
      valid_offsets<NW>(P.N, d, valid);
#pragma unroll
      for (int w = 0; w < NW; ++w)
        gw[w] = far ? valid[w] : ((uint32_t)L.mask2[mi<NW>(L, lane, w)] & valid[w]);
    }
    have_gw = true;
  }
#pragma unroll
  for (int w = 0; w < NW; ++w) L.mask2[mi<NW>(L, lane, w)] = 0ull;
  if (QUEUE && ROWS) L.x1keep[lane] = 0u;
  __syncthreads();
  unsigned long long m2r = 0ull;
  bool queued = false;
  if (QUEUE) {
    static_assert(!QUEUE || NW == 1, "the pair list belongs to one wave");
    const bool far = active && L.far[el] != 0;
    if (active && !have_gw) {
      const int o0 = el * 2 * N + d;
      uint32_t valid[NW];
      valid_offsets<NW>(N, d, valid);
      gw[0] = far ? valid[0]
                  : (gate_word<false>(P, L, o0, 0, H, L.w[WX][o0], L.w[WY][o0], L.w[WZ][o0], L.w[WR][o0]) & valid[0]);
    }
    have_gw = true;
    if (!RVO3D_ABLATED(64 | 128)) queued = x1_queue<ROWS, TOUCH>(P, L, lane, N, active, far, zero_act || act0, gw[0]);
  }
  if (active && !queued) {
    const int o0 = el * 2 * N + d, os0 = el * N + d;
    const float mex = L.w[WX][o0], mey = L.w[WY][o0], mez = L.w[WZ][o0];
    const float mvx = L.w[WVX][os0], mvy = L.w[WVY][os0], mvz = L.w[WVZ][os0];
    const float mer = L.w[WR][o0], mkd = L.w[WKD][os0], mprio = L.w[WPRIO][os0];
    const float max_ = zero_act ? 0.f : L.w[WAX][os0], may = zero_act ? 0.f : L.w[WAY][os0],
                maz = zero_act ? 0.f : L.w[WAZ][os0];
    const bool far = L.far[el] != 0;
    uint32_t valid[NW];
    valid_offsets<NW>(N, d, valid);
    if (ROWS && !TOUCH) RVO3D_STAMP(10);
    if (!have_gw) {
#pragma unroll
      for (int w = 0; w < NW; ++w)
        gw[w] = far ? valid[w] : (gate_word<false>(P, L, o0, w, H, mex, mey, mez, mer) & valid[w]);
    }
    if (ROWS && !TOUCH) RVO3D_STAMP(11);
    const X1End me = {{mex, mex}, {mey, mey}, {mez, mez}, {mer, mer}, {mvx, mvx},
                      {mvy, mvy}, {mvz, mvz}, {mkd, mkd}, {mprio, mprio}};
    const v2f tax = {4.f * max_, 4.f * max_}, tay = {4.f * may, 4.f * may},
              taz = {4.f * maz, 4.f * maz};
#ifndef RVO3D_X1_CW
#define RVO3D_X1_CW 4
#endif
    constexpr int CW = NW < RVO3D_X1_CW ? NW : RVO3D_X1_CW;
#pragma unroll
    for (int w = 0; w < NW / CW; ++w) {
      OffsetSet<CW> cand = OffsetSet<CW>::load(gw + CW * w);
      if (RVO3D_ABLATED(64)) cand = OffsetSet<CW>::none();
      OffsetSet<CW> keep = OffsetSet<CW>::none();
#ifdef RVO3D_DIAG
      if (P.dbg && ROWS && RVO3D_ABLATED(128)) {
        const int c = cand.count();
        atomicAdd(&P.dbg[(size_t)blockIdx.x * 32 + 24], (unsigned long long)c);
        atomicMax(&P.dbg[(size_t)blockIdx.x * 32 + 25], (unsigned long long)c);
      }
#endif
      while (cand.any()) {
        const int kb0 = cand.lowest();
        cand.drop();
        const bool two = cand.any();
        const int kb1 = two ? cand.lowest() : kb0;
        cand.drop();
        const int off0 = 32 * CW * w + kb0 + 1, off1 = 32 * CW * w + kb1 + 1;
        const int oa = o0 + off0, ob = o0 + off1;
        int jd0 = d + off0, jd1 = d + off1;
        if (jd0 >= N) jd0 -= N;
        if (jd1 >= N) jd1 -= N;
        const int ja = el * N + jd0, jb = el * N + jd1;
#define RVO3D_LD2(K, i0, i1) ((v2f){L.w[K][i0], L.w[K][i1]})
        const X1End o = {RVO3D_LD2(WX, oa, ob), RVO3D_LD2(WY, oa, ob), RVO3D_LD2(WZ, oa, ob),
                         RVO3D_LD2(WR, oa, ob), RVO3D_LD2(WVX, ja, jb), RVO3D_LD2(WVY, ja, jb),
                         RVO3D_LD2(WVZ, ja, jb), RVO3D_LD2(WKD, ja, jb), RVO3D_LD2(WPRIO, ja, jb)};
        const v2f z2 = {0.f, 0.f};
        const v2f ajx = zero_act ? z2 : RVO3D_LD2(WAX, ja, jb),
                  ajy = zero_act ? z2 : RVO3D_LD2(WAY, ja, jb),
                  ajz = zero_act ? z2 : RVO3D_LD2(WAZ, ja, jb);
#undef RVO3D_LD2
        const X1Bits xb = x1_pairs<TOUCH, false>(P, far, me, o, tax, tay, taz, ajx, ajy, ajz);
        bool pi0 = xb.pi0, pj0 = xb.pj0, pi1 = xb.pi1, pj1 = xb.pj1;
        if (ROWS) {
          keep.add(kb0, (int)xb.keep0);
          keep.add(kb1, (int)xb.keep1);
        }
        pi1 &= two; pj1 &= two;
        if (NW == 1) {
          m2r |= ((unsigned long long)pi0 << jd0) | ((unsigned long long)pi1 << jd1);
        } else {
          if (pi0) atomicOr(&L.mask2[mi<NW>(L, lane, jd0 >> 6)], 1ull << (jd0 & 63));
          if (pi1) atomicOr(&L.mask2[mi<NW>(L, lane, jd1 >> 6)], 1ull << (jd1 & 63));
        }
        if (pj0) atomicOr(&L.mask2[mi<NW>(L, el * N + jd0, d >> 6)], 1ull << (d & 63));
        if (pj1) atomicOr(&L.mask2[mi<NW>(L, el * N + jd1, d >> 6)], 1ull << (d & 63));
      }
      if (ROWS) keep.store(gw + CW * w);
    }
  }
  if (ROWS && !TOUCH) RVO3D_STAMP(12);
  if (!ROWS) RVO3D_STAMP(14);
  __syncthreads();
  if (QUEUE && ROWS && queued && active) gw[0] = L.x1keep[lane];
#ifdef RVO3D_DIAG
  if (P.dbg && active && RVO3D_ABLATED(128)) {
    int c = 0;
    for (int w = 0; w < NW; ++w) c += __builtin_popcountll(L.mask2[mi<NW>(L, lane, w)] | (w == 0 ? m2r : 0ull));
    atomicAdd(&P.dbg[(size_t)blockIdx.x * 32 + (ROWS ? 22 : 20)], (unsigned long long)c);
    atomicMax(&P.dbg[(size_t)blockIdx.x * 32 + (ROWS ? 23 : 21)], (unsigned long long)c);
  }
#endif
  if (active && !RVO3D_ABLATED(32)) {
    const int lbase = el * N;
#pragma unroll
    for (int w = 0; w < NW; ++w) {
      unsigned long long m2 = L.mask2[mi<NW>(L, lane, w)] | (w == 0 ? m2r : 0ull);
      while (m2) {
        const int j = 64 * w + __builtin_ctzll(m2);
        m2 &= m2 - 1;
        const PairOut po = pair_eval<TRAIN>(P, S, L, lbase + j, a);
        if (TOUCH && po.collision) collision = true;
        if (po.flag) {
          flag = true;
          if (po.t < tmin) tmin = po.t;
          if (ROWS && P.nm > 0) kept = insert_row(P, L, g, lbase, S, po, j, kept);
        }
      }
    }
  }
  if (ROWS && !TOUCH) RVO3D_STAMP(13);
  if (!ROWS) RVO3D_STAMP(15);
  return kept;
}

template <int NW, bool TRAIN, bool GSHARE = false>
__device__ __forceinline__ bool collide_env(const Params& P, const Lds& L, int lane, int el,
                                            int d, bool active, const Drone& S,
                                            uint32_t gw[NW]) {
  const int N = P.N, H = N >> 1;
  uint32_t touchw[NW];
  if (GSHARE) {
    const bool far = L.far[el] != 0;
    if (!far) {
      if (P.uniform_rp) gate_words_shared<NW, true, true>(P, L, d);
      else gate_words_shared<NW, true, false>(P, L, d);
    }
    __syncthreads();
#pragma unroll
    for (int w = 0; w < NW; ++w) {
      const unsigned long long v = L.mask2[mi<NW>(L, lane, w)];
      gw[w] = (uint32_t)v;
      touchw[w] = (uint32_t)(v >> 32);
      if (w) L.mask2[mi<NW>(L, lane, w)] = 0ull;
    }
  }
  L.mask2[mi<NW>(L, lane, 0)] = 0ull;
  __syncthreads();
  bool coll = false;
  if (active) {
    const int o0 = el * 2 * N + d;
    const float mex = L.w[WX][o0], mey = L.w[WY][o0], mez = L.w[WZ][o0], mer = L.w[WR][o0];
    const bool far = L.far[el] != 0;
    uint32_t valid[NW];
    valid_offsets<NW>(N, d, valid);
#pragma unroll
    for (int w = 0; w < NW; ++w) {
      uint32_t cand = valid[w];
      if (GSHARE) {
        if (!far) cand = touchw[w] & valid[w];
        gw[w] = far ? valid[w] : (gw[w] & valid[w]);
      } else {
        gw[w] = valid[w];
        if (!far) {
          uint32_t rng;
          cand = (P.uniform_rp ? gate_word<true, true>(P, L, o0, w, H, mex, mey, mez, mer, &rng)
                               : gate_word<true, false>(P, L, o0, w, H, mex, mey, mez, mer, &rng)) & valid[w];
          gw[w] = rng & valid[w];
        }
      }
      while (cand) {
        const int kb = __builtin_ctz(cand);
        cand &= cand - 1;
        int jd = d + 32 * w + kb + 1;
        if (jd >= N) jd -= N;
        const int k = el * N + jd;
        const double rx = L.x[k] - S.x, ry = L.y[k] - S.y, rz = L.z[k] - S.z;
        const double d2 = dot3b(rx, ry, rz, rx, ry, rz);
        if (!(d2 <= P.T10)) continue;
        if (d2 == 0.0 && rx == 0.0 && ry == 0.0 && rz == 0.0) continue;
        const double Or = L.r[k];
        const double dis = __builtin_sqrt(sq(ry) + sq(rx) + sq(rz));
        bool ci, cj;
        if (TRAIN) {
          ci = cj = dis <= S.r + Or;
        } else {
          ci = dis <= S.r - kExpRadius + Or;
          cj = dis <= Or - kExpRadius + S.r;
          const double R = S.r + Or;
          if (d2 < R * R * (1.0 + 1e-12) && __builtin_sqrt(d2) < R) {
            const bool ai = !ci && S.vx * rx + S.vy * ry + S.vz * rz > 0;
            const bool aj = !cj && L.vx[k] * -rx + L.vy[k] * -ry + L.vz[k] * -rz > 0;
            if (ai || aj) atomicOr(P.err, 2u);
          }
        }
        if (ci) coll = true;
        if (cj) atomicOr(&L.mask2[mi<NW>(L, k, 0)], 1ull);
      }
    }
  }
  __syncthreads();
  if (active && (L.mask2[mi<NW>(L, lane, 0)] & 1ull)) coll = true;
  return coll;
}

__device__ __forceinline__ uint32_t regate_resets(const Params& P, const Lds& L, int tid, int el,
                                                  int d, bool active,
                                                  unsigned long long reset_lanes, uint32_t gw) {
  const int N = P.N, H = N >> 1;
  uint32_t valid[1];
  valid_offsets<1>(N, d, valid);
  const int o0 = el * 2 * N + d;
  const float mex = L.w[WX][o0], mey = L.w[WY][o0], mez = L.w[WZ][o0];
  while (reset_lanes) {
    const int rl = __builtin_ctzll(reset_lanes);
    reset_lanes &= reset_lanes - 1;
    const int rel = __builtin_amdgcn_readlane(el, rl), rd = __builtin_amdgcn_readlane(d, rl);
    const int orr = rel * 2 * N + rd;
    const float dx = L.w[WX][orr] - mex, dy = L.w[WY][orr] - mey, dz = L.w[WZ][orr] - mez;
    const bool same = active && el == rel && tid != rl;
    const bool inr = same && __builtin_signbit(gate_acc(dx, dy, dz, P.t10n));
    int k = rd - d;
    if (k < 0) k += N;
    if (same && k >= 1 && k <= H) {
      const uint32_t bit = 1u << (k - 1);
      gw = (gw & ~bit) | ((inr ? bit : 0u) & valid[0]);
    }
    const unsigned long long bal = __ballot(inr);
    if (tid == rl) {
      unsigned long long seg = bal >> (rel * N), rot;
      if (N == 64) {
        const int sh = (rd + 1) & 63;
        rot = sh ? ((seg >> sh) | (seg << (64 - sh))) : seg;
      } else {
        seg &= (1ull << N) - 1ull;
        const int sh = rd + 1;
        rot = ((seg >> sh) | (seg << (N - sh))) & ((1ull << N) - 1ull);
      }
      gw = (uint32_t)rot & valid[0];
    }
  }
  return gw;
}

}
```

### 3drvo-marl-collisionavoidance_amd/csrc/rvo3d_params.hpp

```cpp
#pragma once

#include <hip/hip_runtime.h>
#include <stdint.h>

namespace rvo3d {

constexpr double kExpRadius = 0.2;
constexpr double kCtimeThreshold = 2.0;
constexpr double kDeg2Rad = 0.017453292519943295;
constexpr double kPi = 3.141592653589793;
constexpr int kMaxThreads = 512;
constexpr double kCosD = 0.999999995;
constexpr double kSinD = 1.0000000000e-4;

struct Cold {
  double map[3];
  double T5, T04;
  double cen[3];
  double act_scale;
  float cmax;
  float kdot;
  uint32_t zf_div;
  uint32_t zf_magic;
  uint32_t zf_q;
  int zf_iters;
  uint32_t zmask[128];
  int nb;
  const double* bld;
  const double* pow95;
  const uint16_t* bgrid;
  int bgx, bgy;
  double bg_inv;
};
constexpr int kBgridK = 15;
typedef const __attribute__((address_space(4))) Cold ColdC;

struct Params {
  int E, N, P, nm, env_train, epb, W;
  int action_f64;
  int dv_cached;
  int g_cached;
  int action_mode;
  float acceler;
#ifdef RVO3D_DIAG
  int ablate;
#endif
  int zf16;
  int uniform_rp;
  double r0, prio0;
  double T10;
  float t10n;
  float bandn;
  float band;
  int nw;
  float x1_gap;
  float x1_k2;
  float x1_cs2;
  double* f64;
  int32_t* i32;
  uint8_t* u8;
  uint32_t S;
  enum { F_PX, F_PY, F_PZ, F_VX, F_VY, F_VZ, F_YAW, F_PITCH, F_REAL_LEN, F_MAX_DEV, F_EXTRA_LEN,
         F_CUR, F_PREV = F_CUR + 3,
         F_ROUTE_LEN = F_PREV + 3, F_RADIUS, F_PRIO, F_DEV0, F_WP };
  __host__ __device__ double* f(int k) const { return f64 + (size_t)k * S; }
  __host__ __device__ double* px() const { return f(F_PX); }
  __host__ __device__ double* py() const { return f(F_PY); }
  __host__ __device__ double* pz() const { return f(F_PZ); }
  __host__ __device__ double* vx() const { return f(F_VX); }
  __host__ __device__ double* vy() const { return f(F_VY); }
  __host__ __device__ double* vz() const { return f(F_VZ); }
  __host__ __device__ double* yaw() const { return f(F_YAW); }
  __host__ __device__ double* pitch() const { return f(F_PITCH); }
  __host__ __device__ double* real_len() const { return f(F_REAL_LEN); }
  __host__ __device__ double* max_dev() const { return f(F_MAX_DEV); }
  __host__ __device__ double* extra_len() const { return f(F_EXTRA_LEN); }
  __host__ __device__ int32_t* wp_idx() const { return i32; }
  __host__ __device__ uint8_t* arrive() const { return u8; }
  __host__ __device__ uint8_t* dest() const { return u8 + S; }
  __host__ __device__ double* route_len() const { return f(F_ROUTE_LEN); }
  __host__ __device__ double* radius() const { return f(F_RADIUS); }
  __host__ __device__ double* prio() const { return f(F_PRIO); }
  __host__ __device__ double* dev0() const { return f(F_DEV0); }
  __host__ __device__ double* wp(int k, int c) const { return f(F_WP + 3 * k + c); }
  __host__ __device__ double* cur(int c) const { return f(F_CUR + c); }
  __host__ __device__ double* prev(int c) const { return f(F_PREV + c); }
  __host__ __device__ int32_t* n_points() const { return i32 + S; }
  __host__ __device__ uint32_t* dvk_a() const { return reinterpret_cast<uint32_t*>(i32) + (size_t)2 * S; }
  __host__ __device__ uint32_t* dvk_b() const { return reinterpret_cast<uint32_t*>(i32) + (size_t)3 * S; }
  __host__ __device__ uint32_t* dv0_a() const { return reinterpret_cast<uint32_t*>(i32) + (size_t)4 * S; }
  __host__ __device__ uint32_t* dv0_b() const { return reinterpret_cast<uint32_t*>(i32) + (size_t)5 * S; }
  __host__ __device__ uint32_t* gcache(int w) const { return reinterpret_cast<uint32_t*>(i32) + (size_t)(6 + w) * S; }
  __host__ __device__ double* row_iet(int s) const { return f(F_WP + 3 * P + s); }
  __host__ __device__ uint32_t* row_pk(int s) const {
    return reinterpret_cast<uint32_t*>(i32) + (size_t)(6 + nw + s) * S;
  }
  __host__ __device__ static size_t f64_arrays(int P_, int nm_) { return F_WP + 3 * (size_t)P_ + (nm_ > 0 ? nm_ : 1); }
  __host__ __device__ static size_t i32_arrays(int nm_, int nw_) { return 6 + (size_t)nw_ + (size_t)(nm_ > 0 ? nm_ : 1); }
  uint32_t* err;
  const Cold* cold_;
  __device__ __forceinline__ ColdC& cold() const { return *(ColdC*)cold_; }
#ifdef RVO3D_DIAG
  unsigned long long* dbg;
#endif
  const void* actions;
  float* obs;
  int32_t* vo_count;
  float* reward;
  double* reward64;
  uint8_t *done, *info, *finish, *reset_mask;
  const int32_t* prev_cnt;
};

#ifdef RVO3D_DIAG
#define RVO3D_STAMP(i)                                                                  \
  do {                                                                                  \
    if (P.dbg && threadIdx.x == 0) P.dbg[(size_t)blockIdx.x * 32 + (i)] = __builtin_amdgcn_s_memtime(); \
  } while (0)
#define RVO3D_ABLATED(bits) ((P.ablate & (bits)) != 0)
#else
#define RVO3D_STAMP(i) do { } while (0)
#define RVO3D_ABLATED(bits) false
#endif

}
```

### 3drvo-marl-collisionavoidance_amd/csrc/rvo3d_step.hpp

```cpp
#pragma once

#include "rvo3d_pairs.hpp"

namespace rvo3d {

__device__ __forceinline__ bool building_test(const double* const bld, int b, const Drone& S,
                                              double T5) {
  const double bx = bld[4 * b], by = bld[4 * b + 1], bh = bld[4 * b + 2], br = bld[4 * b + 3];
  const double ex = S.x - bx, ey = S.y - by;
  if ((bh > S.z - 2) & (norm2sq(ex, ey) <= T5) & (S.z <= bh))
    return __builtin_sqrt(sq(ex) + sq(ey)) <= S.r + br;
  return false;
}
__device__ __forceinline__ bool building_hit(const Params& P, const Drone& S) {
  const int nb = P.cold().nb;
  if (nb == 0) return false;
  bool hit = false;
  const double* const bld = P.cold().bld;
  const double T5 = P.cold().T5;
  const int gx = P.cold().bgx;
  if (gx > 0) {
    const int gy = P.cold().bgy;
    const double inv = P.cold().bg_inv;
    int ix = (int)__builtin_floor(S.x * inv), iy = (int)__builtin_floor(S.y * inv);
    ix = ix < 0 ? 0 : (ix > gx - 1 ? gx - 1 : ix);
    iy = iy < 0 ? 0 : (iy > gy - 1 ? gy - 1 : iy);
    const uint16_t* const cell = P.cold().bgrid + (size_t)(ix * gy + iy) * (kBgridK + 1);
    const uint4 c0 = *reinterpret_cast<const uint4*>(cell);
    const int cnt = (int)(c0.x & 0xffffu);
    if (cnt != 0xffff) {
      if (cnt >= 1) {
        const int b0 = (int)(c0.x >> 16), b1 = cnt >= 2 ? (int)(c0.y & 0xffffu) : b0;
        hit |= building_test(bld, b0, S, T5);
        hit |= building_test(bld, b1, S, T5);
      }
      if (cnt >= 3) {
        const int b0 = (int)(c0.y >> 16), b1 = cnt >= 4 ? (int)(c0.z & 0xffffu) : b0;
        hit |= building_test(bld, b0, S, T5);
        hit |= building_test(bld, b1, S, T5);
      }
      for (int k = 5; k <= cnt; ++k) hit |= building_test(bld, (int)cell[k], S, T5);
      return hit;
    }
  }
#pragma unroll 4
  for (int b = 0; b < nb; ++b) hit |= building_test(bld, b, S, T5);
  return hit;
}

struct ProprioTail { float dv0, dv1, dv2, dev; bool bad; };
__device__ __forceinline__ ProprioTail proprio_tail(const double dv[3], double dev) {
  ProprioTail t;
  t.dv0 = round2_f32(dv[0]); t.dv1 = round2_f32(dv[1]); t.dv2 = round2_f32(dv[2]);
  t.dev = round2_f32(dev);
  t.bad = !(finite_d(dv[0]) && finite_d(dv[1]) && finite_d(dv[2]) && finite_d(dev));
  asm volatile("" : "+v"(t.dv0), "+v"(t.dv1), "+v"(t.dv2), "+v"(t.dev));
  return t;
}
__device__ __forceinline__ void write_proprio(const Params& P, int g, const Drone& S,
                                              const ProprioTail& t) {
  float* o = P.obs + (size_t)g * P.W;
  const double v[8] = {S.x, S.y, S.z, S.vx, S.vy, S.vz, S.r, S.prio};
  float f[12];
  bool bad = t.bad;
#pragma unroll
  for (int k = 0; k < 8; ++k) {
    f[k] = round2_f32(v[k]);
    bad |= !finite_d(v[k]);
  }
  f[8] = t.dv0; f[9] = t.dv1; f[10] = t.dv2; f[11] = t.dev;
  if ((P.W & 1) == 0) {
    float2* o2 = reinterpret_cast<float2*>(o);
#pragma unroll
    for (int k = 0; k < 6; ++k) o2[k] = make_float2(f[2 * k], f[2 * k + 1]);
  } else {
#pragma unroll
    for (int k = 0; k < 12; ++k) o[k] = f[k];
  }
  if (bad) atomicOr(P.err, 1u);
}

__device__ __forceinline__ void stage_row(const Params& P, const Lds& L, int tid, int g,
                                          const Drone& S, const ProprioTail& t, int kept) {
  const double v[8] = {S.x, S.y, S.z, S.vx, S.vy, S.vz, S.r, S.prio};
  float f[12];
  bool bad = t.bad;
#pragma unroll
  for (int k = 0; k < 8; ++k) {
    f[k] = round2_f32(v[k]);
    bad |= !finite_d(v[k]);
  }
  f[8] = t.dv0; f[9] = t.dv1; f[10] = t.dv2; f[11] = t.dev;
  float4* pro = reinterpret_cast<float4*>(L.w[0]) + 3 * tid;
  pro[0] = make_float4(f[0], f[1], f[2], f[3]);
  pro[1] = make_float4(f[4], f[5], f[6], f[7]);
  pro[2] = make_float4(f[8], f[9], f[10], f[11]);
  L.kept[tid] = ((12 + 9 * kept + 1) & ~1) >> 1;
  if (((9 * kept) & 1) && kept < P.nm) P.obs[(size_t)g * P.W + 12 + 9 * kept] = 0.0f;
  if (bad) atomicOr(P.err, 1u);
}

template <int NW>
__device__ __forceinline__ void row_fill_pairs(const Params& P, const Lds& L, int tid, int row0,
                                               int nrows) {
  const int q = P.W >> 1;
  const int ln = tid & 63, wv = tid >> 6;
  const int nwv = NW == 1 ? 1 : (L.T >> 6);
  const int pair0 = row0 >> 1;
  const int npairs = ((row0 + nrows + 1) >> 1) - pair0;
  const int rbase = 2 * pair0 - row0;
  const float2* pro2 = reinterpret_cast<const float2*>(L.w[0]);
  const uint32_t pair_bytes = 8u * (uint32_t)P.W;
  char* const obsb = reinterpret_cast<char*>(P.obs) + (size_t)pair0 * pair_bytes;
  for (int cb = 0; cb < q; cb += 64) {
    const int c = cb + ln;
    const bool lane_on = c < q;
    const int h0 = 2 * c, h1 = 2 * c + 1;
    const int s0 = h0 >= q ? 1 : 0, s1 = h1 >= q ? 1 : 0;
    const int u0 = h0 - (s0 ? q : 0), u1 = h1 - (s1 ? q : 0);
    const bool p0 = u0 < 6, p1 = u1 < 6;
    const int pu0 = p0 ? u0 : 5, pu1 = p1 ? u1 : 5;
    uint32_t off = (uint32_t)wv * pair_bytes + 16u * (uint32_t)c;
    const uint32_t ostep = (uint32_t)nwv * pair_bytes;
    for (int i0 = wv; i0 < npairs; i0 += 4 * nwv) {
      int z0[4], z1[4];
      float2 d0[4], d1[4];
#pragma unroll
      for (int u = 0; u < 4; ++u) {
        const int i = i0 + u * nwv;
        const int lr0 = rbase + 2 * i + s0, lr1 = rbase + 2 * i + s1;
        z0[u] = L.kept[lr0]; z1[u] = L.kept[lr1];
        d0[u] = pro2[lr0 * 6 + pu0]; d1[u] = pro2[lr1 * 6 + pu1];
      }
#pragma unroll
      for (int u = 0; u < 4; ++u) {
        const int i = i0 + u * nwv;
        const int lr0 = rbase + 2 * i + s0, lr1 = rbase + 2 * i + s1;
        const bool live = lane_on & (i < npairs);
        const bool v0 = live & ((unsigned)lr0 < (unsigned)nrows) & (p0 | (u0 >= z0[u]));
        const bool v1 = live & ((unsigned)lr1 < (unsigned)nrows) & (p1 | (u1 >= z1[u]));
        const float2 a = p0 ? d0[u] : make_float2(0.f, 0.f);
        const float2 b = p1 ? d1[u] : make_float2(0.f, 0.f);
        char* const pc = obsb + (off + (uint32_t)u * ostep);
        if (v0 & v1) *reinterpret_cast<float4*>(pc) = make_float4(a.x, a.y, b.x, b.y);
        if (v0 != v1) *reinterpret_cast<float2*>(pc + (v1 ? 8 : 0)) = v1 ? b : a;
      }
      off += 4u * ostep;
    }
  }
}

__device__ __forceinline__ bool two_phase_rows(const Params& P, int row0, int nrows, int full_rows) {
  return P.zf16 && P.cold().zf_iters > 0 && nrows == full_rows && (row0 & 7) == 0;
}

template <int NW>
__device__ __forceinline__ void early_zero_blocks(const Params& P, const Lds& L, int tid, int row0,
                                                  int nrows) {
  const uint32_t rb = 4u * (uint32_t)P.W;
  const int ln = tid & 63, wv = tid >> 6;
  const int nwv = NW == 1 ? 1 : (L.T >> 6);
  (void)nrows;
  char* const base = reinterpret_cast<char*>(P.obs) + (size_t)row0 * rb;
  const uint32_t blk = (uint32_t)wv * 16u + ((uint32_t)ln >> 2);
  typedef float v4f __attribute__((ext_vector_type(4)));
  const int iters = P.cold().zf_iters;
  uint32_t m = P.cold().zmask[tid >> 2];
  if (P.prev_cnt) {
    const bool any = NW == 1 ? __ballot(L.kept[tid] != 0) != 0
                             : __builtin_amdgcn_readfirstlane(*L.any_old) != 0;
    if (!any) return;
    const float inv_rb = 1.0f / (float)rb;
    const uint32_t st = 1024u * (uint32_t)nwv;
    uint32_t keep = 0;
    for (int i = 0; i < iters; ++i)
      if ((m >> i) & 1u) {
        const uint32_t o = blk * 64u + (uint32_t)i * st;
        const uint32_t r = (uint32_t)((float)o * inv_rb);
        if (o - r * rb < 48u + 36u * (uint32_t)L.kept[r]) keep |= 1u << i;
      }
    m = keep;
  }
  char* p = base + (size_t)blk * 64u + 16u * ((uint32_t)ln & 3u);
  const size_t step = (size_t)1024 * (size_t)nwv;
  for (int i = 0; i < iters; i += 4, p += 4 * step, m >>= 4) {
#pragma unroll
    for (int u = 0; u < 4; ++u)
      if ((m >> u) & 1u) {
#if RVO3D_ZERO_NT
        __builtin_nontemporal_store((v4f){0.f, 0.f, 0.f, 0.f}, reinterpret_cast<v4f*>(p + u * step));
#else
        *reinterpret_cast<v4f*>(p + u * step) = (v4f){0.f, 0.f, 0.f, 0.f};
#endif
      }
  }
}

template <int NW>
__device__ __forceinline__ void late_row_windows(const Params& P, const Lds& L, int tid, int row0,
                                                 int nrows) {
  const uint32_t rb = 4u * (uint32_t)P.W, q = rb >> 3;
  const int ln = tid & 63, wv = tid >> 6;
  const int nwv = NW == 1 ? 1 : (L.T >> 6);
  const float2* pro2 = reinterpret_cast<const float2*>(L.w[0]);
  char* const base = reinterpret_cast<char*>(P.obs) + (size_t)row0 * rb;
  const int ch = ln & 7;
  const int r0 = wv * 8 + (ln >> 3);
  const uint32_t rs0 = rb * (uint32_t)r0;
  const uint32_t s8 = (rs0 & 63u) >> 3;
  const uint32_t ua = 2u * (uint32_t)ch, ub = ua + 1u;
  const bool pa = ua < s8, pb = ub < s8;
  const uint32_t uia = pa ? q - s8 + ua : ua - s8, uib = pb ? q - s8 + ub : ub - s8;
  const bool proa = uia < 6u, prob = uib < 6u;
  const int pia = (int)(proa ? uia : 5u), pib = (int)(prob ? uib : 5u);
  const int da_row = pa ? 1 : 0, db_row = pb ? 1 : 0;
  char* pc = base + (rs0 & ~63u) + 16u * (uint32_t)ch;
  const size_t step = (size_t)8 * (size_t)nwv * rb;
  for (int r = r0; r < nrows; r += 8 * nwv, pc += step) {
    const int ra = r - da_row, rbw = r - db_row;
    const int za = L.kept[ra], zb = L.kept[rbw];
    const float2 da = pro2[ra * 6 + pia], db = pro2[rbw * 6 + pib];
    const bool va = proa | (uia >= (uint32_t)za), vb = prob | (uib >= (uint32_t)zb);
    const float2 a = proa ? da : make_float2(0.f, 0.f), b = prob ? db : make_float2(0.f, 0.f);
    if (va & vb) *reinterpret_cast<float4*>(pc) = make_float4(a.x, a.y, b.x, b.y);
    if (va != vb) *reinterpret_cast<float2*>(pc + (vb ? 8 : 0)) = vb ? b : a;
  }
}

__device__ __forceinline__ void write_vo_rows(const Params& P, const Lds& L, int tid, int lbase,
                                              int g, const Drone& S, int kept) {
  float* o = P.obs + (size_t)g * P.W;
  bool bad = false;
  for (int s = 0; s < kept; ++s) {
    const uint32_t pk = P.row_pk(s)[g];
    const int j = (int)(pk & 0xffffu);
    const Drone O = lds_drone(L, lbase + j);
    const double pr = (S.prio == O.prio) ? 0.5 : S.prio / (S.prio + O.prio);
    double row[9];
    row[0] = pr * (2 * S.x + (S.vx + O.vx));
    row[1] = pr * (2 * S.y + (S.vy + O.vy));
    row[2] = pr * (2 * S.z + (S.vz + O.vz));
    row[3] = O.x - S.x; row[4] = O.y - S.y; row[5] = O.z - S.z;
    row[6] = (double)(pk >> 16) / 100.0;
    row[7] = pair_md(S, O);
    row[8] = P.row_iet(s)[g];
#pragma unroll
    for (int k = 0; k < 9; ++k) {
      bad |= !finite_d(row[k]);
      o[12 + 9 * s + k] = round2_f32(row[k]);
    }
  }
  P.vo_count[g] = kept;
  if (bad) atomicOr(P.err, 1u);
}

__device__ __forceinline__ void publish_zero_run(const Params& P, int g, int kept) {
  if ((P.W & 1) == 0 && ((9 * kept) & 1) && kept < P.nm) P.obs[(size_t)g * P.W + 12 + 9 * kept] = 0.0f;
}

__device__ __forceinline__ void zero_fill(const Params& P, const Lds& L, int tid, int row0,
                                          int nrows) {
  const uint32_t per_row = P.cold().zf_div;
  if (per_row == 0) return;
  const uint32_t total = (uint32_t)nrows * per_row;
  float* base = P.obs + (size_t)row0 * P.W + 12;
  if ((P.W & 1) == 0) {
    for (uint32_t q = tid; q < total; q += L.T) {
      const uint32_t row = (uint32_t)(((uint64_t)q * P.cold().zf_magic) >> 32);
      const uint32_t c = q - row * per_row;
      const uint32_t first = (9u * (uint32_t)L.kept[row] + 1u) >> 1;
      if (c >= first)
        *reinterpret_cast<float2*>(base + (size_t)row * P.W + 2 * c) = make_float2(0.f, 0.f);
    }
  } else {
    for (uint32_t q = tid; q < total; q += L.T) {
      const uint32_t row = (uint32_t)(((uint64_t)q * P.cold().zf_magic) >> 32);
      const uint32_t c = q - row * per_row;
      if (c >= 9u * (uint32_t)L.kept[row]) base[(size_t)row * P.W + c] = 0.0f;
    }
  }
}

__device__ __forceinline__ void load_wp(const Params& P, int g, int k, double out[3]) {
  out[0] = P.wp(k, 0)[g];
  out[1] = P.wp(k, 1)[g];
  out[2] = P.wp(k, 2)[g];
}

__device__ __forceinline__ void load3(double* const a0, double* const a1, double* const a2, int g,
                                      double out[3]) {
  out[0] = a0[g]; out[1] = a1[g]; out[2] = a2[g];
}
__device__ __forceinline__ void store3(double* const a0, double* const a1, double* const a2, int g,
                                       const double v[3]) {
  a0[g] = v[0]; a1[g] = v[1]; a2[g] = v[2];
}
#define RVO3D_LOAD_CUR(P, g, out) load3((P).cur(0), (P).cur(1), (P).cur(2), g, out)
#define RVO3D_LOAD_PREV(P, g, out) load3((P).prev(0), (P).prev(1), (P).prev(2), g, out)
#define RVO3D_STORE_CUR(P, g, v) store3((P).cur(0), (P).cur(1), (P).cur(2), g, v)
#define RVO3D_STORE_PREV(P, g, v) store3((P).prev(0), (P).prev(1), (P).prev(2), g, v)

__device__ __forceinline__ double rvo_reward_pre(const double dv[3], const double a[3]) {
  const double d0 = dv[0], d1 = dv[1], d2 = dv[2];
  const double vel_penalty = 0.2 * norm3b(a[0], a[1], a[2]) / norm3b(d0, d1, d2);
  const double eps = 1e-8;
  const double magA = __builtin_sqrt(sq(d0) + sq(d1) + sq(d2) + eps);
  const double magB = __builtin_sqrt(sq(a[0]) + sq(a[1]) + sq(a[2]) + eps);
  const double dotp = d0 * a[0] + d1 * a[1] + d2 * a[2];
  double c = dotp / (magA * magB);
  c = c < -1.0 + eps ? -1.0 + eps : (c > 1.0 - eps ? 1.0 - eps : c);
  const double C18 = 0.984807753012208, C6 = 0.8660254037844387, C3 = 0.5000000000000001,
               C2 = 6.123233995736766e-17;
  double punish;
  if (c == 0.0) punish = -4;
  else if (__builtin_fabs(c - C18) > 1e-12 && __builtin_fabs(c - C6) > 1e-12 &&
           __builtin_fabs(c - C3) > 1e-12 && __builtin_fabs(c - C2) > 1e-12) {
    punish = c > C18 ? 3 : (c > C6 ? 1 : (c > C3 ? 0.5 : (c > C2 ? 0 : -4)));
    if (c != c) punish = -4;
  } else {
    const double ang = acos(c);
    if (ang < kPi / 18) punish = 3;
    else if (ang < kPi / 6) punish = 1;
    else if (ang < kPi / 3) punish = 0.5;
    else if (ang < kPi / 2) punish = 0;
    else punish = -4;
  }
  return punish + vel_penalty;
}
__device__ __forceinline__ double rvo_reward_k(double pre, bool flag, double tmin) {
  double safety = 0;
  if (flag) {
    double urgency = 0;
    if (tmin < 2) urgency = -8.0 * exp(-tmin / 0.5);
    safety = -2.5 + urgency;
  }
  return __builtin_rint((pre + safety) * 1000.0);
}

__device__ __forceinline__ double mov_reward_k(const Params& P, bool collision, bool arrive_r,
                                               int waypoint_num, int n_points_m1, bool dest_r,
                                               double dev, bool len_flag, double exlen) {
  if (collision) return -50000.0;
  double reward = 0;
  if (arrive_r) reward += 3.0 * P.cold().pow95[n_points_m1 - waypoint_num];
  if (dest_r) reward += 20.0;
  const double d = dev * 10;
  const double dev_pen = -1.5 * (2 / (1 + exp(-(d - 5) / 0.3)));
  double ex_pen = 0;
  if (len_flag) {
    ex_pen = -0.3 * log(exlen + 1 + 1e-6);
    if (ex_pen < -6 || ex_pen != ex_pen) ex_pen = -6;
  }
  return __builtin_rint((reward + dev_pen + ex_pen) * 1000.0);
}


enum Mode { kObserve = 0, kStep = 1, kStepAutoReset = 2 };

#ifndef RVO3D_ZERO_NT
#define RVO3D_ZERO_NT 1
#endif
#ifndef RVO3D_DEPHASE
#define RVO3D_DEPHASE 0
#endif

#ifndef RVO3D_WAVES_ATTR
#define RVO3D_WAVES_ATTR __attribute__((amdgpu_waves_per_eu(NW <= 4 ? 4 : 3)))
#endif

template <int MODE, int NW, int NFIX = 0, bool TRAIN = true, bool PAD = (NFIX != 0 && NW > 1)>
__global__ void __launch_bounds__(64 * NW) RVO3D_WAVES_ATTR env_kernel(const Params Pin) {
  extern __shared__ __attribute__((aligned(16))) unsigned char smem[];
  Params P = Pin;
  static_assert(!PAD || NFIX != 0, "a padded kernel has a compile-time ring size");
  const int Nr = Pin.N;
  if (NFIX) { P.N = NFIX; P.epb = NFIX <= 64 ? 64 / NFIX : 1; }
  const int tid = threadIdx.x, T = (NW == 1 || NFIX) ? 64 * NW : (int)blockDim.x, N = P.N;
  const Lds L = carve_lds(smem, T, P.nm, P.epb, N, NW);
  const int el = tid / N;
  const int d = tid - el * N;
  const int e0 = blockIdx.x * P.epb;
  const int e = e0 + el;
  const bool active = (el < P.epb) && (e < P.E) && (!PAD || d < Nr);
  const int g = active ? e * (PAD ? Nr : N) + d : 0;
  const int lbase = el * N;
  const int full_rows = P.epb * (PAD ? Nr : N);
  const int nrows = ((P.E - e0) < P.epb ? (P.E - e0) : P.epb) * (PAD ? Nr : N);
  const int row0 = e0 * (PAD ? Nr : N);
  const int lrow = PAD ? el * Nr + d : tid;
  constexpr bool LITE = (MODE == kStepAutoReset);
  constexpr bool GSH = NW > 1 && NFIX == 64 * NW;
  constexpr bool XQ = NW == 1 && NFIX != 0;

  RVO3D_STAMP(0);
#if RVO3D_DEPHASE
  if (NW == 1) {
    unsigned hw_slot;
    asm volatile("s_getreg_b32 %0, hwreg(HW_REG_HW_ID)" : "=s"(hw_slot));
    if (hw_slot & 1)
      for (int i = 0; i < RVO3D_DEPHASE; ++i) __builtin_amdgcn_s_sleep(32);
  }
#endif
  Drone S;
  S.x = S.y = S.z = S.vx = S.vy = S.vz = 0.0; S.r = 0.2; S.prio = 5;
  if (PAD && d >= Nr) {
    S.x = S.y = S.z = __builtin_inf();
    const int o = el * 2 * N + d, os = el * N + d;
#pragma unroll
    for (int k = 0; k < 12; ++k) {
      const float v = (k == WX || k == WY || k == WZ) ? 1e30f : (k == WKD ? -1.0f : 0.0f);
      if (k == WX || k == WY || k == WZ || k == WR) {
        L.w[k][o] = v;
        if (d <= (N >> 1)) L.w[k][o + N] = v;
      } else L.w[k][os] = v;
    }
  }
  double a[3] = {0, 0, 0}, cur[3] = {0, 0, 0}, dv[3] = {0, 0, 0};
  double dev = 0, max_dev = 0;
  int wpi = 1;

  uint32_t gw[NW];
  const bool have_gw = MODE != kObserve && P.g_cached != 0;
  uint32_t old_cnt = 0;
  if (active) {
    if (LITE && NW == 1 && P.prev_cnt) {
      old_cnt = (uint32_t)P.prev_cnt[g];
      old_cnt = old_cnt < (uint32_t)P.nm ? old_cnt : (uint32_t)P.nm;
    }
    S.x = P.px()[g]; S.y = P.py()[g]; S.z = P.pz()[g];
    S.vx = P.vx()[g]; S.vy = P.vy()[g]; S.vz = P.vz()[g];
    if (P.uniform_rp) { S.r = P.r0; S.prio = P.prio0; }
    else { S.r = P.radius()[g]; S.prio = P.prio()[g]; }
    if (have_gw) {
#pragma unroll
      for (int w = 0; w < NW; ++w) gw[w] = P.gcache(w)[g];
    }
    if (MODE != kObserve) {
      if (P.action_mode == 1) {
        const float* A = static_cast<const float*>(P.actions) + (size_t)g * 3;
        const double vv[3] = {S.vx, S.vy, S.vz};
#pragma unroll
        for (int k = 0; k < 3; ++k) {
          const float r = __builtin_rintf(A[k] * 100.0f) / 100.0f;
          const double x = (double)(P.acceler * r) + vv[k];
          a[k] = __builtin_rint(x * 100.0) / 100.0;
        }
      } else {
        if (P.action_f64) {
          const double* A = static_cast<const double*>(P.actions) + (size_t)g * 3;
          a[0] = A[0]; a[1] = A[1]; a[2] = A[2];
        } else {
          const float* A = static_cast<const float*>(P.actions) + (size_t)g * 3;
          a[0] = (double)A[0]; a[1] = (double)A[1]; a[2] = (double)A[2];
        }
        if (P.cold().act_scale > 0) {
          a[0] = __builtin_rint(a[0] * P.cold().act_scale) / P.cold().act_scale;
          a[1] = __builtin_rint(a[1] * P.cold().act_scale) / P.cold().act_scale;
          a[2] = __builtin_rint(a[2] * P.cold().act_scale) / P.cold().act_scale;
        }
      }
    }
  }
  RVO3D_STAMP(1);
  double az[3] = {a[0], a[1], a[2]};
  if (norm3b(a[0], a[1], a[2]) < 1e-5) az[0] = az[1] = az[2] = 0.0;
  const double zero3[3] = {0, 0, 0};

  if (tid < P.epb) { L.any_reset[tid] = 0; L.far[tid] = 0; }
  if (LITE && NW > 1 && tid == 0) *L.any_old = 0;
  L.kept[tid] = 0;
  __syncthreads();
  if (LITE && NW == 1 && active && P.prev_cnt) L.kept[lrow] = (int)old_cnt;
  L.x[tid] = S.x; L.y[tid] = S.y; L.z[tid] = S.z;
  L.vx[tid] = S.vx; L.vy[tid] = S.vy; L.vz[tid] = S.vz;
  L.r[tid] = S.r; L.prio[tid] = S.prio;
  {
    const double p[3] = {S.x, S.y, S.z}, v[3] = {S.vx, S.vy, S.vz};
    stage_f32<NW>(P, L, el, d, active, p, v, az, S.r, S.prio);
  }
  __syncthreads();

  bool flag, collision = false;
  double tmin;

  if (MODE == kObserve) {
    if (active) {
      double prev[3];
      max_dev = P.max_dev()[g];
      RVO3D_LOAD_CUR(P, g, cur);
      RVO3D_LOAD_PREV(P, g, prev);
      const double p[3] = {S.x, S.y, S.z};
      des_vel(P, p, cur, dv);
      dev = deviation(prev, cur, p);
      if (dev > max_dev) max_dev = dev;
    }
    const int kept = sweep_env<NW, true, true, TRAIN, GSH, XQ>(P, L, tid, el, d, g, active, S, zero3, true, true, flag,
                                               tmin, collision, gw, false);
    if (active) {
      write_vo_rows(P, L, tid, lbase, g, S, kept);
      if (P.zf16) stage_row(P, L, lrow, g, S, proprio_tail(dv, dev), kept);
      else {
        write_proprio(P, g, S, proprio_tail(dv, dev));
        publish_zero_run(P, g, kept);
        L.kept[lrow] = kept;
      }
      P.max_dev()[g] = max_dev;
      uint32_t dvk_a, dvk_b;
      dv_encode(dv, dvk_a, dvk_b);
      P.dvk_a()[g] = dvk_a; P.dvk_b()[g] = dvk_b;
#pragma unroll
      for (int w = 0; w < NW; ++w) P.gcache(w)[g] = gw[w];
    }
    __syncthreads();
    if (P.zf16) row_fill_pairs<NW>(P, L, tid, row0, nrows);
    else zero_fill(P, L, tid, row0, nrows);
    return;
  }

  RVO3D_STAMP(2);
  sweep_env<NW, false, false, TRAIN, GSH, XQ>(P, L, tid, el, d, g, active && !RVO3D_ABLATED(1), S, az, false, false, flag,
                              tmin, collision, gw, have_gw);
  double rew_k = 0;
  double mov_nc = 0;
  bool f_dest = false;
  RVO3D_STAMP(3);
  constexpr bool kLoadAhead = NW <= 2;
  double prev[3] = {0, 0, 0}, yaw = 0, pitch = 0, real_len = 0, route_len = 0;
  int npts = 2;
  bool f_arrive_in = false, f_dest_in = false;
#define RVO3D_LOAD_INTEGRATION_STATE()                                               \
  {                                                                                  \
    wpi = P.wp_idx()[g];                                                             \
    RVO3D_LOAD_PREV(P, g, prev);                                                     \
    yaw = P.yaw()[g]; pitch = P.pitch()[g]; real_len = P.real_len()[g];              \
    route_len = P.route_len()[g];                                                    \
    npts = P.n_points()[g];                                                          \
    f_arrive_in = P.arrive()[g] != 0; f_dest_in = P.dest()[g] != 0;                  \
  }
  if (active) {
    max_dev = P.max_dev()[g];
    RVO3D_LOAD_CUR(P, g, cur);
    uint32_t dvk_a = 0, dvk_b = 0;
    if (P.dv_cached) { dvk_a = P.dvk_a()[g]; dvk_b = P.dvk_b()[g]; }
    if (kLoadAhead) RVO3D_LOAD_INTEGRATION_STATE()
    bool have = false;
    if (P.dv_cached) have = dv_decode(dvk_a, dvk_b, dv);
    if (!have) {
      if (!kLoadAhead) RVO3D_LOAD_PREV(P, g, prev);
      const double p[3] = {S.x, S.y, S.z};
      des_vel(P, p, cur, dv);
      dev = deviation(prev, cur, p);
      if (dev > max_dev) max_dev = dev;
    }
    rew_k = rvo_reward_k(rvo_reward_pre(dv, a), flag, tmin);
  }
  RVO3D_STAMP(18);
  __syncthreads();
  if (active) {
    if (!kLoadAhead) RVO3D_LOAD_INTEGRATION_STATE()
#undef RVO3D_LOAD_INTEGRATION_STATE
    bool ex_set = false;
    double extra_len = 0.0;
    const int wpi_in = wpi;
    bool f_arrive = f_arrive_in;
    f_dest = f_dest_in;

    double speed = norm3b(S.vx, S.vy, S.vz);
    const double acc = clampd(a[0] * 1.0, -1.0, 1.0);
    const double dyaw = clampd(a[1] * 90.0, -90.0, 90.0);
    const double dpit = clampd(a[2] * 90.0, -90.0, 90.0);
    const double nv = speed + acc;
    speed = (0.0 > nv) ? 0.0 : nv;
    yaw = np_mod(yaw + dyaw, 360.0);
    pitch = clampd(pitch + dpit, -90.0, 90.0);
    double nvx = 0.0, nvy = 0.0, nvz = 0.0;
    if (!f_dest) {
      double sy, cy, sp, cp;
      sincos(yaw * kDeg2Rad, &sy, &cy);
      sincos(pitch * kDeg2Rad, &sp, &cp);
      nvx = speed * cp * cy; nvy = speed * cp * sy; nvz = speed * sp;
    }
    const double q0 = S.x, q1 = S.y, q2 = S.z;
    S.x = S.x + nvx; S.y = S.y + nvy; S.z = S.z + nvz;
    S.vx = nvx; S.vy = nvy; S.vz = nvz;
    real_len = real_len + norm3b(S.x - q0, S.y - q1, S.z - q2);
    const double p[3] = {S.x, S.y, S.z};
    double dst[3] = {0, 0, 0};
    if (f_arrive || arrived(P, p, cur)) load_wp(P, g, npts - 1, dst);
    if (arrived(P, p, cur)) {
      const bool at_dst = arrived(P, p, dst);
      if (at_dst) { extra_len = real_len - route_len; ex_set = true; }
      if (!at_dst && wpi < npts - 1) {
        wpi += 1;
        prev[0] = cur[0]; prev[1] = cur[1]; prev[2] = cur[2];
        load_wp(P, g, wpi, cur);
        RVO3D_STORE_CUR(P, g, cur);
        RVO3D_STORE_PREV(P, g, prev);
        f_arrive = false;
      }
    }
    des_vel(P, p, cur, dv);
    dev = deviation(prev, cur, p);
    if (dev > max_dev) max_dev = dev;
    bool arrive_r = false, dest_r = false;
    const int waypoint_num = wpi;
    if (!f_arrive && arrived(P, p, cur)) { f_arrive = true; arrive_r = true; }
    if (f_arrive) {
      if (arrived(P, p, dst)) {
        extra_len = real_len - route_len;
        ex_set = true;
        if (!f_dest) { f_dest = true; dest_r = true; }
      }
    }
    const double exlen = real_len - route_len + 4;
    mov_nc = mov_reward_k(P, false, arrive_r, waypoint_num, npts - 1, dest_r, dev, exlen > 0,
                          exlen);
    RVO3D_STAMP(19);
    collision = building_hit(P, S);
    if (S.x < 0 || S.x > P.cold().map[0] || S.y < 0 || S.y > P.cold().map[1] || S.z < 0 || S.z > P.cold().map[2])
      collision = true;
    P.yaw()[g] = yaw; P.pitch()[g] = pitch; P.real_len()[g] = real_len;
    if (ex_set) P.extra_len()[g] = extra_len;
    if (wpi != wpi_in) P.wp_idx()[g] = wpi;
    if (f_arrive != f_arrive_in) P.arrive()[g] = f_arrive ? 1 : 0;
    if (f_dest != f_dest_in) P.dest()[g] = f_dest ? 1 : 0;
    P.info[g] = f_arrive ? 1 : 0;
    P.finish[g] = f_dest ? 1 : 0;
  }
  L.x[tid] = S.x; L.y[tid] = S.y; L.z[tid] = S.z;
  L.vx[tid] = S.vx; L.vy[tid] = S.vy; L.vz[tid] = S.vz;
  {
    const double p[3] = {S.x, S.y, S.z}, v[3] = {S.vx, S.vy, S.vz};
    stage_f32<NW>(P, L, el, d, active, p, v, az, S.r, S.prio);
  }
  __syncthreads();

  RVO3D_STAMP(4);
  int kept = 0;
  if (LITE) {
    if (collide_env<NW, TRAIN, GSH>(P, L, tid, el, d, active && !RVO3D_ABLATED(2), S, gw)) collision = true;
  } else {
    kept = sweep_env<NW, true, true, TRAIN, GSH, XQ>(P, L, tid, el, d, g, active && !RVO3D_ABLATED(2), S, az, false,
                                     false, flag, tmin, collision, gw, false);
  }
  bool do_reset = false;
  if (active) {
    const double rew64 = k_over_1000(rew_k) + k_over_1000(collision ? -50000.0 : mov_nc);
    P.reward[g] = (float)rew64;
    if (P.reward64) P.reward64[g] = rew64;
    P.done[g] = collision ? 1 : 0;
    do_reset = LITE && (collision || f_dest);
  }

  RVO3D_STAMP(5);
  if (LITE) {
    if (active && P.reset_mask) P.reset_mask[g] = do_reset ? 1 : 0;
    if (do_reset) L.any_reset[el] = 1;
    __syncthreads();
    double p[3] = {0, 0, 0}, rcur[3] = {0, 0, 0}, rdev = 0.0;
    uint32_t rdv_a = 0, rdv_b = 0;
    if (NW > 1 && active && P.prev_cnt) {
      old_cnt = (uint32_t)P.prev_cnt[g];
      old_cnt = old_cnt < (uint32_t)P.nm ? old_cnt : (uint32_t)P.nm;
      L.kept[lrow] = (int)old_cnt;
      if (old_cnt != 0) *L.any_old = 1;
    }
    if (do_reset) {
      load_wp(P, g, 0, p);
      rdev = P.dev0()[g];
      load_wp(P, g, 1, rcur);
      rdv_a = P.dv0_a()[g]; rdv_b = P.dv0_b()[g];
    }
    RVO3D_STAMP(26);
    if (NW == 1 && two_phase_rows(P, row0, nrows, full_rows) && !RVO3D_ABLATED(16)) early_zero_blocks<NW>(P, L, tid, row0, nrows);
    RVO3D_STAMP(27);
    if (do_reset) {
      S.x = p[0]; S.y = p[1]; S.z = p[2]; S.vx = S.vy = S.vz = 0.0;
      dev = rdev;
      cur[0] = rcur[0]; cur[1] = rcur[1]; cur[2] = rcur[2];
      if (!dv_decode(rdv_a, rdv_b, dv)) {
        des_vel(P, p, cur, dv);
        dev = deviation(p, cur, p);
      }
      RVO3D_STORE_CUR(P, g, cur);
      RVO3D_STORE_PREV(P, g, p);
      max_dev = dev > 0.0 ? dev : 0.0;
      P.wp_idx()[g] = 1; P.arrive()[g] = 0; P.dest()[g] = 0;
      P.real_len()[g] = 0.0; P.yaw()[g] = 0.0; P.pitch()[g] = 0.0;
      L.x[tid] = S.x; L.y[tid] = S.y; L.z[tid] = S.z;
      L.vx[tid] = 0.0; L.vy[tid] = 0.0; L.vz[tid] = 0.0;
      const double v0[3] = {0, 0, 0};
      stage_f32<NW>(P, L, el, d, true, p, v0, az, S.r, S.prio);
    }
    if (active && L.any_reset[el] != 0) {
      const int os = el * N + d;
      L.w[WAX][os] = 0.f; L.w[WAY][os] = 0.f; L.w[WAZ][os] = 0.f;
    }
  }
  if (active) {
    uint32_t dvk_a, dvk_b;
    dv_encode(dv, dvk_a, dvk_b);
    P.dvk_a()[g] = dvk_a; P.dvk_b()[g] = dvk_b;
  }
  const ProprioTail ptail = proprio_tail(dv, dev);
  if (active) P.max_dev()[g] = max_dev;
  if (LITE) {
    __syncthreads();
    RVO3D_STAMP(6);
    const bool env_reset = (active || (PAD && el < P.epb)) && (L.any_reset[el] != 0);
    bool c2 = false;
    const double aa[3] = {env_reset ? 0.0 : az[0], env_reset ? 0.0 : az[1], env_reset ? 0.0 : az[2]};
    bool have_gw2 = !env_reset;
    if (NW == 1) {
      const unsigned long long rlanes = __ballot(do_reset);
      if (L.far[el] != 0) {
        uint32_t valid[1];
        valid_offsets<1>(N, d, valid);
        gw[0] = valid[0];
      } else {
        gw[0] = regate_resets(P, L, tid, el, d, active, rlanes, gw[0]);
      }
      have_gw2 = true;
    }
    if (RVO3D_ABLATED(2)) have_gw2 = false;
    if (NW > 1 && two_phase_rows(P, row0, nrows, full_rows) && !RVO3D_ABLATED(16)) early_zero_blocks<NW>(P, L, tid, row0, nrows);
    kept = sweep_env<NW, true, false, TRAIN, GSH, XQ>(P, L, tid, el, d, g, active && !RVO3D_ABLATED(4), S, aa,
                                      false, env_reset, flag, tmin, c2, gw, have_gw2);
  }
  RVO3D_STAMP(7);
  const bool two_phase = LITE && two_phase_rows(P, row0, nrows, full_rows);
  if (NW > 1 && two_phase) {
    asm volatile("s_waitcnt vmcnt(0)" ::: "memory");
    __syncthreads();
  }
  if (active) {
    if (!RVO3D_ABLATED(8)) {
      if (two_phase) asm volatile("s_waitcnt vmcnt(0)" ::: "memory");
      write_vo_rows(P, L, tid, lbase, g, S, kept);
      RVO3D_STAMP(16);
      if (P.zf16) stage_row(P, L, lrow, g, S, ptail, kept);
      else { write_proprio(P, g, S, ptail); publish_zero_run(P, g, kept); }
    }
    if (!P.zf16) L.kept[lrow] = kept;
  }
  __syncthreads();
  RVO3D_STAMP(17);
  if (!RVO3D_ABLATED(16)) {
    if (two_phase) late_row_windows<NW>(P, L, tid, row0, nrows);
    else if (P.zf16) row_fill_pairs<NW>(P, L, tid, row0, nrows);
    else zero_fill(P, L, tid, row0, nrows);
  }
  RVO3D_STAMP(8);
  if (active) {
#pragma unroll
    for (int w = 0; w < NW; ++w) P.gcache(w)[g] = gw[w];
    P.px()[g] = S.x; P.py()[g] = S.y; P.pz()[g] = S.z;
    P.vx()[g] = S.vx; P.vy()[g] = S.vy; P.vz()[g] = S.vz;
  }
  RVO3D_STAMP(9);
}

}
```

Before: 7.813 billion drone-steps/s.

## Move hot constants into kernel arguments and hoist action loads for single-wave path

Splits the device-side constant block into a Hot struct carried inside the kernel argument Params, so the NW==1 path reads thresholds, map bounds, centre, act_scale and pow95 from the kernarg segment instead of dereferencing the global Cold pointer. It also re-reads those values from the kernarg pointer at points of use to limit scalar register pressure. Action words and prev_cnt are loaded early as raw 32-bit words so their latency overlaps the state loads. The cost is a larger kernarg block and more code complexity, and prev_cnt now falls back to reading wp_idx when absent, with the clamp moved to its later use.

```diff
diff --git a/3drvo-marl-collisionavoidance_amd/csrc/rvo3d_capi.hip b/3drvo-marl-collisionavoidance_amd/csrc/rvo3d_capi.hip
--- a/3drvo-marl-collisionavoidance_amd/csrc/rvo3d_capi.hip
+++ b/3drvo-marl-collisionavoidance_amd/csrc/rvo3d_capi.hip
@@ -82,7 +82,7 @@
       {(void**)&P.i32, ni * S * 4},
       {(void**)&P.u8, 2 * S},
       {(void**)&C.bld, (size_t)(c.num_buildings > 0 ? c.num_buildings : 1) * 4 * 8},
-      {(void**)&C.pow95, (size_t)c.max_points * 8},
+      {(void**)&P.hot_.pow95, (size_t)c.max_points * 8},
       {(void**)&C.bgrid, (size_t)(C.bgx > 0 ? C.bgx * C.bgy : 1) * (rvo3d::kBgridK + 1) * 2},
       {(void**)&P.err, 256},
       {(void**)&P.cold_, sizeof(rvo3d::Cold)},
@@ -97,6 +97,7 @@
     *x.slot = static_cast<char*>(h->arena) + off;
     off += align_up(x.bytes, 256);
   }
+  C.hot = P.hot_;
   HIP_TRY(hipMemcpy((void*)P.cold_, &C, sizeof C, hipMemcpyHostToDevice));
   return RVO3D_OK;
 }
@@ -367,13 +368,13 @@
   std::memset(&P, 0, sizeof P);
   std::memset(&C, 0, sizeof C);
   P.E = cfg->num_envs; P.N = cfg->num_drones; P.P = cfg->max_points;
-  C.nb = cfg->num_buildings; P.nm = cfg->neighbors_num; P.env_train = cfg->env_train ? 1 : 0;
+  P.hot_.nb = cfg->num_buildings; P.nm = cfg->neighbors_num; P.env_train = cfg->env_train ? 1 : 0;
   P.W = 12 + 9 * P.nm;
 #ifdef RVO3D_DIAG
   if (const char* ab = std::getenv("RVO3D_ABLATE")) P.ablate = std::atoi(ab);
 #endif
-  C.act_scale = cfg->action_decimals >= 0 ? std::pow(10.0, cfg->action_decimals) : 0.0;
-  for (int k = 0; k < 3; ++k) C.map[k] = cfg->map_size[k];
+  P.hot_.act_scale = cfg->action_decimals >= 0 ? std::pow(10.0, cfg->action_decimals) : 0.0;
+  for (int k = 0; k < 3; ++k) P.hot_.map[k] = cfg->map_size[k];
   P.T10 = sq_threshold(10.0);
   C.T5 = sq_threshold(5.0);
   C.bgx = C.bgy = 0; C.bg_inv = 0.0;
@@ -385,21 +386,21 @@
     if (C.bgy < 1) C.bgy = 1;
     C.bg_inv = 1.0 / cs;
   }
-  C.T04 = sq_threshold(0.4);
+  P.hot_.T04 = sq_threshold(0.4);
   {
-    double mx = std::fmax(C.map[0], std::fmax(C.map[1], C.map[2]));
+    double mx = std::fmax(P.hot_.map[0], std::fmax(P.hot_.map[1], P.hot_.map[2]));
     if (!(mx > 0)) mx = 1.0;
-    for (int k = 0; k < 3; ++k) C.cen[k] = 0.5 * C.map[k];
+    for (int k = 0; k < 3; ++k) P.hot_.cen[k] = 0.5 * P.hot_.map[k];
     const double cmax = 0.75 * mx + 16.0;
     const double u = std::ldexp(1.0, -24);
     const double eD = u * (2.0 * cmax + 21.0);
     const double band = 2.0 * (2.0 * 1.7320508 * 10.5 * eD + 3.0 * eD * eD + 8.0 * u * 110.25);
-    C.cmax = (float)cmax;
+    P.hot_.cmax = (float)cmax;
     P.band = std::nextafter((float)band, INFINITY);
     const float t10f = std::nextafter((float)(P.T10 + band), INFINITY);
     P.t10n = -std::nextafter(t10f, INFINITY);
     P.bandn = P.band + P.t10n;
-    C.kdot = std::nextafter((float)(2.0 * (eD + 4.0 * u * 10.5) * 1.001), INFINITY);
+    P.hot_.kdot = std::nextafter((float)(2.0 * (eD + 4.0 * u * 10.5) * 1.001), INFINITY);
     const double gap = 512.0 * band;
     const double cs = 4.0 * (1.7320508 * eD / std::sqrt(gap) + 8.0 * u);
     P.x1_gap = (float)gap;
@@ -436,7 +437,7 @@
     C.zf_magic = m;
   }
   C.zf_q = (P.W & 1) == 0 ? (uint32_t)(P.W / 2) : 0u;
-  C.zf_iters = 0;
+  P.hot_.zf_iters = 0;
   static_assert(rvo3d::kMaxThreads / 4 <= sizeof(C.zmask) / sizeof(C.zmask[0]),
                 "Cold::zmask has one word per thread quad of the largest workgroup");
   std::memset(C.zmask, 0, sizeof C.zmask);
@@ -456,7 +457,7 @@
         }
         C.zmask[tq] = m;
       }
-      C.zf_iters = (int)iters;
+      P.hot_.zf_iters = (int)iters;
     }
   }
   h->threads = threads;
@@ -498,7 +499,7 @@
   if (!waypoints || !n_points) return fail(RVO3D_ERR_INVALID, "waypoints / n_points are required");
   const Params& P = h->P;
   const rvo3d::Cold& C = h->cold;
-  if (C.nb > 0 && !buildings) return fail(RVO3D_ERR_INVALID, "buildings required when num_buildings > 0");
+  if (P.hot_.nb > 0 && !buildings) return fail(RVO3D_ERR_INVALID, "buildings required when num_buildings > 0");
   hipStream_t s = static_cast<hipStream_t>(stream);
   const size_t EN = (size_t)P.E * P.N;
   std::vector<double> wp((size_t)P.P * 3 * EN), rl(EN), rad(EN), pri(EN), p95(P.P);
@@ -535,10 +536,10 @@
   HIP_TRY(hipMemcpyAsync((void*)P.route_len(), rl.data(), EN * 8, hipMemcpyHostToDevice, s));
   HIP_TRY(hipMemcpyAsync((void*)P.radius(), rad.data(), EN * 8, hipMemcpyHostToDevice, s));
   HIP_TRY(hipMemcpyAsync((void*)P.prio(), pri.data(), EN * 8, hipMemcpyHostToDevice, s));
-  HIP_TRY(hipMemcpyAsync((void*)C.pow95, p95.data(), (size_t)P.P * 8, hipMemcpyHostToDevice, s));
+  HIP_TRY(hipMemcpyAsync((void*)P.hot_.pow95, p95.data(), (size_t)P.P * 8, hipMemcpyHostToDevice, s));
   std::vector<uint16_t> grid;
-  if (C.nb > 0) {
-    HIP_TRY(hipMemcpyAsync((void*)C.bld, buildings, (size_t)C.nb * 32, hipMemcpyHostToDevice, s));
+  if (P.hot_.nb > 0) {
+    HIP_TRY(hipMemcpyAsync((void*)C.bld, buildings, (size_t)P.hot_.nb * 32, hipMemcpyHostToDevice, s));
     if (C.bgx > 0) {
       const int K = rvo3d::kBgridK;
       const double cs = 1.0 / C.bg_inv;
@@ -555,7 +556,7 @@
           const double y0 = iy == 0 ? -INFINITY : iy * cs, y1 = iy == C.bgy - 1 ? INFINITY : (iy + 1) * cs;
           int n = 0;
           bool overflow = false;
-          for (int b = 0; b < C.nb && !overflow; ++b) {
+          for (int b = 0; b < P.hot_.nb && !overflow; ++b) {
             const double bx = buildings[4 * b], by = buildings[4 * b + 1];
             double reach = rmax + buildings[4 * b + 3];
             if (!(reach < 5.0)) reach = 5.0;
diff --git a/3drvo-marl-collisionavoidance_amd/csrc/rvo3d_math.hpp b/3drvo-marl-collisionavoidance_amd/csrc/rvo3d_math.hpp
--- a/3drvo-marl-collisionavoidance_amd/csrc/rvo3d_math.hpp
+++ b/3drvo-marl-collisionavoidance_amd/csrc/rvo3d_math.hpp
@@ -72,11 +72,12 @@
   return m;
 }
 
+template <bool ARGS = true>
 __device__ __forceinline__ void des_vel(const Params& P, const double p[3], const double cur[3],
                                         double out[3]) {
   const double dx = cur[0] - p[0], dy = cur[1] - p[1], dz = cur[2] - p[2];
   const double d2 = dot3b(dx, dy, dz, dx, dy, dz);
-  if (d2 > P.cold().T04) {
+  if (d2 > P.hot<ARGS>().T04) {
     const double inv = 1000.0 / __builtin_sqrt(d2);
     const double ux = dx * inv, uy = dy * inv, uz = dz * inv;
     double kx = __builtin_rint(ux), ky = __builtin_rint(uy), kz = __builtin_rint(uz);
@@ -111,9 +112,10 @@
   return __builtin_sqrt(sq(p[0] - qx) + sq(p[1] - qy) + sq(p[2] - qz));
 }
 
+template <bool ARGS = true>
 __device__ __forceinline__ bool arrived(const Params& P, const double p[3], const double d[3]) {
   const double x = p[0] - d[0], y = p[1] - d[1], z = p[2] - d[2];
-  return dot3b(x, y, z, x, y, z) <= P.cold().T04;
+  return dot3b(x, y, z, x, y, z) <= P.hot<ARGS>().T04;
 }
 
 __device__ __forceinline__ double vo_exp_time(double rx, double ry, double rz, double rvx,
diff --git a/3drvo-marl-collisionavoidance_amd/csrc/rvo3d_pairs.hpp b/3drvo-marl-collisionavoidance_amd/csrc/rvo3d_pairs.hpp
--- a/3drvo-marl-collisionavoidance_amd/csrc/rvo3d_pairs.hpp
+++ b/3drvo-marl-collisionavoidance_amd/csrc/rvo3d_pairs.hpp
@@ -120,12 +120,13 @@
                                           bool active, const double p[3], const double v[3],
                                           const double az[3], double r, double prio) {
   if (!active) return;
-  const double cx = p[0] - P.cold().cen[0], cy = p[1] - P.cold().cen[1], cz = p[2] - P.cold().cen[2];
+  const auto& H = P.hot<NW == 1>();
+  const double cx = p[0] - H.cen[0], cy = p[1] - H.cen[1], cz = p[2] - H.cen[2];
   const float fvx = (float)v[0], fvy = (float)v[1], fvz = (float)v[2];
   const bool vzero = v[0] == 0.0 && v[1] == 0.0 && v[2] == 0.0;
   const float val[12] = {(float)cx, (float)cy, (float)cz, fvx, fvy, fvz, (float)r,
                          vzero ? -1.0f
-                               : P.cold().kdot * (__builtin_fabsf(fvx) + __builtin_fabsf(fvy) + __builtin_fabsf(fvz)) + 1e-30f,
+                               : H.kdot * (__builtin_fabsf(fvx) + __builtin_fabsf(fvy) + __builtin_fabsf(fvz)) + 1e-30f,
                          (float)az[0], (float)az[1], (float)az[2], (float)prio};
   const int o = el * 2 * P.N + d, os = el * P.N + d;
 #pragma unroll
@@ -135,7 +136,7 @@
       if (NW == 1 || d <= (P.N >> 1)) L.w[k][o + P.N] = val[k];
     } else L.w[k][os] = val[k];
   }
-  const double cm = (double)P.cold().cmax;
+  const double cm = (double)H.cmax;
   if (!(__builtin_fabs(cx) <= cm && __builtin_fabs(cy) <= cm && __builtin_fabs(cz) <= cm))
     L.far[el] = 1;
 }
diff --git a/3drvo-marl-collisionavoidance_amd/csrc/rvo3d_params.hpp b/3drvo-marl-collisionavoidance_amd/csrc/rvo3d_params.hpp
--- a/3drvo-marl-collisionavoidance_amd/csrc/rvo3d_params.hpp
+++ b/3drvo-marl-collisionavoidance_amd/csrc/rvo3d_params.hpp
@@ -13,21 +13,26 @@
 constexpr double kCosD = 0.999999995;
 constexpr double kSinD = 1.0000000000e-4;
 
-struct Cold {
+struct Hot {
+  double T04;
   double map[3];
-  double T5, T04;
+  double act_scale;
   double cen[3];
-  double act_scale;
   float cmax;
   float kdot;
+  int nb;
+  int zf_iters;
+  const double* pow95;
+};
+
+struct Cold {
+  Hot hot;
+  double T5;
   uint32_t zf_div;
   uint32_t zf_magic;
   uint32_t zf_q;
-  int zf_iters;
   uint32_t zmask[128];
-  int nb;
   const double* bld;
-  const double* pow95;
   const uint16_t* bgrid;
   int bgx, bgy;
   double bg_inv;
@@ -49,6 +54,7 @@
   int uniform_rp;
   double r0, prio0;
   double T10;
+  Hot hot_;
   float t10n;
   float bandn;
   float band;
@@ -100,6 +106,11 @@
   uint32_t* err;
   const Cold* cold_;
   __device__ __forceinline__ ColdC& cold() const { return *(ColdC*)cold_; }
+  template <bool ARGS>
+  __device__ __forceinline__ const auto& hot() const {
+    if constexpr (ARGS) return hot_;
+    else return cold().hot;
+  }
 #ifdef RVO3D_DIAG
   unsigned long long* dbg;
 #endif
@@ -111,6 +122,24 @@
   uint8_t *done, *info, *finish, *reset_mask;
   const int32_t* prev_cnt;
 };
+
+typedef const __attribute__((address_space(4))) Params ParamsC;
+__device__ __forceinline__ ParamsC& kernarg_again() {
+  ParamsC* k = (ParamsC*)__builtin_amdgcn_kernarg_segment_ptr();
+  asm volatile("" : "+s"(k));
+  return *k;
+}
+__device__ __forceinline__ void reread_goal(Params& P) { P.hot_.T04 = kernarg_again().hot_.T04; }
+__device__ __forceinline__ void reread_map(Params& P) {
+  ParamsC& Q = kernarg_again();
+  P.hot_.map[0] = Q.hot_.map[0]; P.hot_.map[1] = Q.hot_.map[1]; P.hot_.map[2] = Q.hot_.map[2];
+  P.hot_.nb = Q.hot_.nb;
+}
+__device__ __forceinline__ void reread_stage(Params& P) {
+  ParamsC& Q = kernarg_again();
+  P.hot_.cen[0] = Q.hot_.cen[0]; P.hot_.cen[1] = Q.hot_.cen[1]; P.hot_.cen[2] = Q.hot_.cen[2];
+  P.hot_.cmax = Q.hot_.cmax; P.hot_.kdot = Q.hot_.kdot;
+}
 
 #ifdef RVO3D_DIAG
 #define RVO3D_STAMP(i)                                                                  \
diff --git a/3drvo-marl-collisionavoidance_amd/csrc/rvo3d_step.hpp b/3drvo-marl-collisionavoidance_amd/csrc/rvo3d_step.hpp
--- a/3drvo-marl-collisionavoidance_amd/csrc/rvo3d_step.hpp
+++ b/3drvo-marl-collisionavoidance_amd/csrc/rvo3d_step.hpp
@@ -12,8 +12,9 @@
     return __builtin_sqrt(sq(ex) + sq(ey)) <= S.r + br;
   return false;
 }
+template <bool ARGS>
 __device__ __forceinline__ bool building_hit(const Params& P, const Drone& S) {
-  const int nb = P.cold().nb;
+  const int nb = P.hot<ARGS>().nb;
   if (nb == 0) return false;
   bool hit = false;
   const double* const bld = P.cold().bld;
@@ -150,8 +151,9 @@
   }
 }
 
+template <bool ARGS>
 __device__ __forceinline__ bool two_phase_rows(const Params& P, int row0, int nrows, int full_rows) {
-  return P.zf16 && P.cold().zf_iters > 0 && nrows == full_rows && (row0 & 7) == 0;
+  return P.zf16 && (ARGS ? kernarg_again().hot_.zf_iters : P.cold().hot.zf_iters) > 0 && nrows == full_rows && (row0 & 7) == 0;
 }
 
 template <int NW>
@@ -164,12 +166,13 @@
   char* const base = reinterpret_cast<char*>(P.obs) + (size_t)row0 * rb;
   const uint32_t blk = (uint32_t)wv * 16u + ((uint32_t)ln >> 2);
   typedef float v4f __attribute__((ext_vector_type(4)));
-  const int iters = P.cold().zf_iters;
-  uint32_t m = P.cold().zmask[tid >> 2];
+  const int iters = NW == 1 ? kernarg_again().hot_.zf_iters : P.cold().hot.zf_iters;
+  uint32_t m;
   if (P.prev_cnt) {
     const bool any = NW == 1 ? __ballot(L.kept[tid] != 0) != 0
                              : __builtin_amdgcn_readfirstlane(*L.any_old) != 0;
     if (!any) return;
+    m = P.cold().zmask[tid >> 2];
     const float inv_rb = 1.0f / (float)rb;
     const uint32_t st = 1024u * (uint32_t)nwv;
     uint32_t keep = 0;
@@ -180,6 +183,8 @@
         if (o - r * rb < 48u + 36u * (uint32_t)L.kept[r]) keep |= 1u << i;
       }
     m = keep;
+  } else {
+    m = P.cold().zmask[tid >> 2];
   }
   char* p = base + (size_t)blk * 64u + 16u * ((uint32_t)ln & 3u);
   const size_t step = (size_t)1024 * (size_t)nwv;
@@ -337,12 +342,13 @@
   return __builtin_rint((pre + safety) * 1000.0);
 }
 
+template <bool ARGS>
 __device__ __forceinline__ double mov_reward_k(const Params& P, bool collision, bool arrive_r,
                                                int waypoint_num, int n_points_m1, bool dest_r,
                                                double dev, bool len_flag, double exlen) {
   if (collision) return -50000.0;
   double reward = 0;
-  if (arrive_r) reward += 3.0 * P.cold().pow95[n_points_m1 - waypoint_num];
+  if (arrive_r) reward += 3.0 * (ARGS ? kernarg_again().hot_.pow95 : P.cold().hot.pow95)[n_points_m1 - waypoint_num];
   if (dest_r) reward += 20.0;
   const double d = dev * 10;
   const double dev_pen = -1.5 * (2 / (1 + exp(-(d - 5) / 0.3)));
@@ -391,6 +397,7 @@
   constexpr bool LITE = (MODE == kStepAutoReset);
   constexpr bool GSH = NW > 1 && NFIX == 64 * NW;
   constexpr bool XQ = NW == 1 && NFIX != 0;
+  constexpr bool KA = NW == 1;
 
   RVO3D_STAMP(0);
 #if RVO3D_DEPHASE
@@ -423,9 +430,17 @@
   const bool have_gw = MODE != kObserve && P.g_cached != 0;
   uint32_t old_cnt = 0;
   if (active) {
-    if (LITE && NW == 1 && P.prev_cnt) {
-      old_cnt = (uint32_t)P.prev_cnt[g];
-      old_cnt = old_cnt < (uint32_t)P.nm ? old_cnt : (uint32_t)P.nm;
+    if (LITE && NW == 1) {
+      const int32_t* const pc = P.prev_cnt ? P.prev_cnt : P.wp_idx();
+      old_cnt = (uint32_t)pc[g];
+    }
+    uint32_t aw[6] = {0, 0, 0, 0, 0, 0};
+    const bool a64 = MODE != kObserve && P.action_mode != 1 && P.action_f64 != 0;
+    if (MODE != kObserve && KA) {
+      const uint32_t* const A = static_cast<const uint32_t*>(P.actions) + (size_t)g * (a64 ? 6 : 3);
+      const uint32_t* const A2 = A + (a64 ? 3 : 0);
+      aw[0] = A[0]; aw[1] = A[1]; aw[2] = A[2];
+      aw[3] = A2[0]; aw[4] = A2[1]; aw[5] = A2[2];
     }
     S.x = P.px()[g]; S.y = P.py()[g]; S.z = P.pz()[g];
     S.vx = P.vx()[g]; S.vy = P.vy()[g]; S.vz = P.vz()[g];
@@ -435,7 +450,7 @@
 #pragma unroll
       for (int w = 0; w < NW; ++w) gw[w] = P.gcache(w)[g];
     }
-    if (MODE != kObserve) {
+    if (MODE != kObserve && !KA) {
       if (P.action_mode == 1) {
         const float* A = static_cast<const float*>(P.actions) + (size_t)g * 3;
         const double vv[3] = {S.vx, S.vy, S.vz};
@@ -453,10 +468,36 @@
           const float* A = static_cast<const float*>(P.actions) + (size_t)g * 3;
           a[0] = (double)A[0]; a[1] = (double)A[1]; a[2] = (double)A[2];
         }
-        if (P.cold().act_scale > 0) {
-          a[0] = __builtin_rint(a[0] * P.cold().act_scale) / P.cold().act_scale;
-          a[1] = __builtin_rint(a[1] * P.cold().act_scale) / P.cold().act_scale;
-          a[2] = __builtin_rint(a[2] * P.cold().act_scale) / P.cold().act_scale;
+        if (P.cold().hot.act_scale > 0) {
+          a[0] = __builtin_rint(a[0] * P.cold().hot.act_scale) / P.cold().hot.act_scale;
+          a[1] = __builtin_rint(a[1] * P.cold().hot.act_scale) / P.cold().hot.act_scale;
+          a[2] = __builtin_rint(a[2] * P.cold().hot.act_scale) / P.cold().hot.act_scale;
+        }
+      }
+    }
+    if (MODE != kObserve && KA) {
+      if (P.action_mode == 1) {
+        const double vv[3] = {S.vx, S.vy, S.vz};
+#pragma unroll
+        for (int k = 0; k < 3; ++k) {
+          const float r = __builtin_rintf(__builtin_bit_cast(float, aw[k]) * 100.0f) / 100.0f;
+          const double x = (double)(P.acceler * r) + vv[k];
+          a[k] = __builtin_rint(x * 100.0) / 100.0;
+        }
+      } else {
+        if (a64) {
+#pragma unroll
+          for (int k = 0; k < 3; ++k)
+            a[k] = __builtin_bit_cast(double, (uint64_t)aw[2 * k] | ((uint64_t)aw[2 * k + 1] << 32));
+        } else {
+#pragma unroll
+          for (int k = 0; k < 3; ++k) a[k] = (double)__builtin_bit_cast(float, aw[k]);
+        }
+        const double sc = P.hot<KA>().act_scale;
+        if (sc > 0) {
+          a[0] = __builtin_rint(a[0] * sc) / sc;
+          a[1] = __builtin_rint(a[1] * sc) / sc;
+          a[2] = __builtin_rint(a[2] * sc) / sc;
         }
       }
     }
@@ -470,7 +511,8 @@
   if (LITE && NW > 1 && tid == 0) *L.any_old = 0;
   L.kept[tid] = 0;
   __syncthreads();
-  if (LITE && NW == 1 && active && P.prev_cnt) L.kept[lrow] = (int)old_cnt;
+  if (LITE && NW == 1 && active && P.prev_cnt)
+    L.kept[lrow] = (int)(old_cnt < (uint32_t)P.nm ? old_cnt : (uint32_t)P.nm);
   L.x[tid] = S.x; L.y[tid] = S.y; L.z[tid] = S.z;
   L.vx[tid] = S.vx; L.vy[tid] = S.vy; L.vz[tid] = S.vz;
   L.r[tid] = S.r; L.prio[tid] = S.prio;
@@ -490,7 +532,7 @@
       RVO3D_LOAD_CUR(P, g, cur);
       RVO3D_LOAD_PREV(P, g, prev);
       const double p[3] = {S.x, S.y, S.z};
-      des_vel(P, p, cur, dv);
+      des_vel<KA>(P, p, cur, dv);
       dev = deviation(prev, cur, p);
       if (dev > max_dev) max_dev = dev;
     }
@@ -537,6 +579,7 @@
     npts = P.n_points()[g];                                                          \
     f_arrive_in = P.arrive()[g] != 0; f_dest_in = P.dest()[g] != 0;                  \
   }
+  if (MODE != kObserve && KA) reread_goal(P);
   if (active) {
     max_dev = P.max_dev()[g];
     RVO3D_LOAD_CUR(P, g, cur);
@@ -548,7 +591,7 @@
     if (!have) {
       if (!kLoadAhead) RVO3D_LOAD_PREV(P, g, prev);
       const double p[3] = {S.x, S.y, S.z};
-      des_vel(P, p, cur, dv);
+      des_vel<KA>(P, p, cur, dv);
       dev = deviation(prev, cur, p);
       if (dev > max_dev) max_dev = dev;
     }
@@ -586,9 +629,9 @@
     real_len = real_len + norm3b(S.x - q0, S.y - q1, S.z - q2);
     const double p[3] = {S.x, S.y, S.z};
     double dst[3] = {0, 0, 0};
-    if (f_arrive || arrived(P, p, cur)) load_wp(P, g, npts - 1, dst);
-    if (arrived(P, p, cur)) {
-      const bool at_dst = arrived(P, p, dst);
+    if (f_arrive || arrived<KA>(P, p, cur)) load_wp(P, g, npts - 1, dst);
+    if (arrived<KA>(P, p, cur)) {
+      const bool at_dst = arrived<KA>(P, p, dst);
       if (at_dst) { extra_len = real_len - route_len; ex_set = true; }
       if (!at_dst && wpi < npts - 1) {
         wpi += 1;
@@ -599,26 +642,29 @@
         f_arrive = false;
       }
     }
-    des_vel(P, p, cur, dv);
+    des_vel<KA>(P, p, cur, dv);
     dev = deviation(prev, cur, p);
     if (dev > max_dev) max_dev = dev;
     bool arrive_r = false, dest_r = false;
     const int waypoint_num = wpi;
-    if (!f_arrive && arrived(P, p, cur)) { f_arrive = true; arrive_r = true; }
+    if (!f_arrive && arrived<KA>(P, p, cur)) { f_arrive = true; arrive_r = true; }
     if (f_arrive) {
-      if (arrived(P, p, dst)) {
+      if (arrived<KA>(P, p, dst)) {
         extra_len = real_len - route_len;
         ex_set = true;
         if (!f_dest) { f_dest = true; dest_r = true; }
       }
     }
     const double exlen = real_len - route_len + 4;
-    mov_nc = mov_reward_k(P, false, arrive_r, waypoint_num, npts - 1, dest_r, dev, exlen > 0,
+    mov_nc = mov_reward_k<KA>(P, false, arrive_r, waypoint_num, npts - 1, dest_r, dev, exlen > 0,
                           exlen);
     RVO3D_STAMP(19);
-    collision = building_hit(P, S);
-    if (S.x < 0 || S.x > P.cold().map[0] || S.y < 0 || S.y > P.cold().map[1] || S.z < 0 || S.z > P.cold().map[2])
-      collision = true;
+    if (KA) reread_map(P);
+    collision = building_hit<KA>(P, S);
+    const auto& H = P.hot<KA>();
+    if (KA) { if ((S.x < 0) | (S.x > H.map[0]) | (S.y < 0) | (S.y > H.map[1]) | (S.z < 0) | (S.z > H.map[2])) collision = true; }
+    else if (S.x < 0 || S.x > H.map[0] || S.y < 0 || S.y > H.map[1] || S.z < 0 || S.z > H.map[2]) collision = true;
+    if (KA) reread_stage(P);
     P.yaw()[g] = yaw; P.pitch()[g] = pitch; P.real_len()[g] = real_len;
     if (ex_set) P.extra_len()[g] = extra_len;
     if (wpi != wpi_in) P.wp_idx()[g] = wpi;
@@ -665,6 +711,7 @@
       L.kept[lrow] = (int)old_cnt;
       if (old_cnt != 0) *L.any_old = 1;
     }
+    if (KA) reread_stage(P);
     if (do_reset) {
       load_wp(P, g, 0, p);
       rdev = P.dev0()[g];
@@ -672,14 +719,15 @@
       rdv_a = P.dv0_a()[g]; rdv_b = P.dv0_b()[g];
     }
     RVO3D_STAMP(26);
-    if (NW == 1 && two_phase_rows(P, row0, nrows, full_rows) && !RVO3D_ABLATED(16)) early_zero_blocks<NW>(P, L, tid, row0, nrows);
+    if (NW == 1 && two_phase_rows<KA>(P, row0, nrows, full_rows) && !RVO3D_ABLATED(16)) early_zero_blocks<NW>(P, L, tid, row0, nrows);
     RVO3D_STAMP(27);
     if (do_reset) {
       S.x = p[0]; S.y = p[1]; S.z = p[2]; S.vx = S.vy = S.vz = 0.0;
       dev = rdev;
       cur[0] = rcur[0]; cur[1] = rcur[1]; cur[2] = rcur[2];
       if (!dv_decode(rdv_a, rdv_b, dv)) {
-        des_vel(P, p, cur, dv);
+        if (KA) reread_goal(P);
+        des_vel<KA>(P, p, cur, dv);
         dev = deviation(p, cur, p);
       }
       RVO3D_STORE_CUR(P, g, cur);
@@ -723,12 +771,12 @@
       have_gw2 = true;
     }
     if (RVO3D_ABLATED(2)) have_gw2 = false;
-    if (NW > 1 && two_phase_rows(P, row0, nrows, full_rows) && !RVO3D_ABLATED(16)) early_zero_blocks<NW>(P, L, tid, row0, nrows);
+    if (NW > 1 && two_phase_rows<KA>(P, row0, nrows, full_rows) && !RVO3D_ABLATED(16)) early_zero_blocks<NW>(P, L, tid, row0, nrows);
     kept = sweep_env<NW, true, false, TRAIN, GSH, XQ>(P, L, tid, el, d, g, active && !RVO3D_ABLATED(4), S, aa,
                                       false, env_reset, flag, tmin, c2, gw, have_gw2);
   }
   RVO3D_STAMP(7);
-  const bool two_phase = LITE && two_phase_rows(P, row0, nrows, full_rows);
+  const bool two_phase = LITE && two_phase_rows<KA>(P, row0, nrows, full_rows);
   if (NW > 1 && two_phase) {
     asm volatile("s_waitcnt vmcnt(0)" ::: "memory");
     __syncthreads();
```

Measured after the change: 8.065 billion drone-steps/s (median of 6 runs). +3.2%, better.
